# angeris/cfmm-routing-code

Hardware: NVIDIA H100
Metric: pools x dual-evaluations / second (1M constant-product pools, 4096 tokens); time to 1e-6 rel-gap reported beside it (higher is better)
Workload: dtype f64

## Files before the change

### cfmm_routing_code_b200/_lib.py

```python
from __future__ import annotations

import ctypes as C
import os

from . import build as _build

KIND_PRODUCT, KIND_SUM, KIND_GEOMEAN, KIND_BOUNDED = 0, 1, 2, 3

_ERRORS = {
    -1: "CFMM_E_NULL (required pointer is NULL)",
    -2: "CFMM_E_KIND (unknown kind / unsupported arity)",
    -3: "CFMM_E_SIZE (bad size)",
    -4: "CFMM_E_CUDA (CUDA runtime error)",
    -5: "CFMM_E_NODEVICE (no sm_90 device)",
    -6: "CFMM_E_STATE (handle used in the wrong state)",
}


class CfmmError(RuntimeError):
    pass


class Bucket(C.Structure):
    _fields_ = [
        ("kind", C.c_int32), ("arity", C.c_int32), ("n_pools", C.c_int64), ("stride", C.c_int64),
        ("reserves", C.c_void_p), ("tok_idx", C.c_void_p), ("gamma", C.c_void_p),
        ("weights", C.c_void_p), ("logrw", C.c_void_p), ("theta_bar", C.c_void_p),
    ]


class BlockedPairs(C.Structure):
    _fields_ = [
        ("n_pools", C.c_int64), ("n_tiles", C.c_int64), ("pools_per_tile", C.c_int32), ("reserved", C.c_int32),
        ("r0", C.c_void_p), ("r1", C.c_void_p), ("gamma_inv", C.c_void_p), ("lid", C.c_void_p),
        ("pos", C.c_void_p), ("rows", C.c_void_p), ("tok", C.c_void_p), ("desc", C.c_void_p),
    ]


class SolveParams(C.Structure):
    _fields_ = [("tol", C.c_double), ("nu_floor", C.c_double), ("max_iter", C.c_int32), ("cg_max", C.c_int32)]


class SolveResult(C.Structure):
    _fields_ = [("dual_value", C.c_double), ("primal_value", C.c_double), ("gap", C.c_double),
                ("primal_infeas", C.c_double), ("err", C.c_double), ("iters", C.c_int32), ("evals", C.c_int32),
                ("hvps", C.c_int32), ("status", C.c_int32)]


class PeerCtx(C.Structure):
    _fields_ = [("recv_acc_dev", C.c_void_p), ("recv_vec_dev", C.c_void_p), ("rank", C.c_int32), ("world", C.c_int32),
                ("seq_acc", C.c_uint64), ("seq_vec", C.c_uint64)]


class CsrPools(C.Structure):
    _fields_ = [("n_tokens", C.c_int32), ("n_pools", C.c_int64), ("nnz", C.c_int64), ("pool_ptr", C.c_void_p),
                ("tok_idx", C.c_void_p), ("reserves", C.c_void_p), ("weights", C.c_void_p), ("logrw", C.c_void_p),
                ("gamma", C.c_void_p), ("kind", C.c_void_p)]


class Batch(C.Structure):
    _fields_ = [("n_problems", C.c_int32), ("pool_range", C.c_void_p), ("c", C.c_void_p), ("a", C.c_void_p),
                ("flags", C.c_void_p), ("nu", C.c_void_p), ("psi", C.c_void_p), ("stats", C.c_void_p),
                ("delta", C.c_void_p), ("lambda_", C.c_void_p), ("trade_stride", C.c_int64)]


class BatchParams(C.Structure):
    _fields_ = [("tol", C.c_double), ("eps0", C.c_double), ("eps_min", C.c_double), ("eps_shrink", C.c_double),
                ("floor_rel", C.c_double), ("max_outer", C.c_int32), ("max_inner", C.c_int32)]


class EvalOut(C.Structure):
    _fields_ = [("delta", C.c_void_p), ("lambda_", C.c_void_p), ("hcoef", C.c_void_p), ("hmask", C.c_void_p)]


_lib = None


def lib_path() -> str:
    return _build.LIB


def load(build_if_missing: bool = True):
    global _lib
    if _lib is not None:
        return _lib
    path = _build.LIB
    if build_if_missing and _build.needs_build():
        try:
            _build.build_library()
        except Exception as e:
            if not os.path.exists(path):
                raise CfmmError(f"libcfmm_b200.so is missing and could not be built: {e}") from e
    if not os.path.exists(path):
        raise CfmmError("libcfmm_b200.so is missing: run `python -c 'import __graft_entry__ as g; g.build()'`")
    lib = C.CDLL(path)
    vp, i32, i64, dbl = C.c_void_p, C.c_int32, C.c_int64, C.c_double
    lib.cfmm_arb_eval.argtypes = [C.POINTER(Bucket), i32, vp, vp, dbl, vp, vp, C.POINTER(EvalOut), vp]
    lib.cfmm_arb_eval.restype = C.c_int
    for name in ("cfmm_hvp", "cfmm_hess_diag", "cfmm_hess_dense"):
        fn = getattr(lib, name)
        fn.restype = C.c_int
    lib.cfmm_hvp.argtypes = [C.POINTER(Bucket), i32, vp, vp, vp, vp, vp]
    lib.cfmm_hess_diag.argtypes = [C.POINTER(Bucket), i32, vp, vp, vp, vp]
    lib.cfmm_hess_dense.argtypes = [C.POINTER(Bucket), i32, vp, vp, vp, vp]
    lib.cfmm_blocked_layout_info.argtypes = [C.POINTER(i32)] * 4
    lib.cfmm_blocked_layout_info.restype = C.c_int
    lib.cfmm_set_blocked_config.argtypes = [i32]
    lib.cfmm_set_blocked_config.restype = C.c_int
    lib.cfmm_blocked_build_work_bytes.argtypes = [i64]
    lib.cfmm_blocked_build_work_bytes.restype = i64
    lib.cfmm_blocked_build.argtypes = [i64, i32, vp, vp, vp, C.POINTER(BlockedPairs), vp, vp, vp, i64, vp]
    lib.cfmm_blocked_build.restype = C.c_int
    lib.cfmm_blocked_eval.argtypes = [C.POINTER(BlockedPairs), i32, vp, vp, vp, C.POINTER(EvalOut), vp, i64, vp]
    lib.cfmm_blocked_eval.restype = C.c_int
    lib.cfmm_blocked_hvp.argtypes = [C.POINTER(BlockedPairs), i32, vp, vp, vp, vp, vp]
    lib.cfmm_blocked_hvp.restype = C.c_int
    lib.cfmm_blocked_diag.argtypes = [C.POINTER(BlockedPairs), i32, vp, vp, vp]
    lib.cfmm_blocked_diag.restype = C.c_int
    lib.cfmm_blocked_dense.argtypes = [C.POINTER(BlockedPairs), i32, vp, vp, vp]
    lib.cfmm_blocked_dense.restype = C.c_int
    lib.cfmm_blocked_solve_work_bytes.argtypes = [C.POINTER(BlockedPairs), i32]
    lib.cfmm_blocked_solve_work_bytes.restype = i64
    lib.cfmm_blocked_solve.argtypes = [C.POINTER(BlockedPairs), i32, vp, vp, vp, vp, vp, vp, vp,
                                       C.POINTER(SolveParams), C.POINTER(SolveResult), vp]
    lib.cfmm_blocked_solve.restype = C.c_int
    lib.cfmm_blocked_solve_peer.argtypes = [C.POINTER(BlockedPairs), i32, vp, vp, vp, vp, vp, vp, vp,
                                            C.POINTER(SolveParams), C.POINTER(SolveResult), C.POINTER(PeerCtx), vp]
    lib.cfmm_blocked_solve_peer.restype = C.c_int
    lib.cfmm_persist_solve_work_bytes.argtypes = [C.POINTER(BlockedPairs), i32]
    lib.cfmm_persist_solve_work_bytes.restype = i64
    lib.cfmm_persist_solve.argtypes = lib.cfmm_blocked_solve_peer.argtypes
    lib.cfmm_persist_solve.restype = C.c_int
    lib.cfmm_set_persist_cooperative.argtypes = [i32]
    lib.cfmm_set_persist_cooperative.restype = C.c_int
    lib.cfmm_persist_last_profile.argtypes = [vp]
    lib.cfmm_persist_last_profile.restype = C.c_int
    lib.cfmm_batch_solve_work_bytes.argtypes = [C.POINTER(CsrPools), i32, i64]
    lib.cfmm_batch_solve_work_bytes.restype = i64
    lib.cfmm_set_batch_lanes.argtypes = [i32]
    lib.cfmm_set_batch_lanes.restype = C.c_int
    lib.cfmm_batch_solve.argtypes = [C.POINTER(CsrPools), C.POINTER(Batch), C.POINTER(BatchParams), vp, vp]
    lib.cfmm_batch_solve.restype = C.c_int
    lib.cfmm_allreduce_ll.argtypes = [vp, vp, i32, i32, i32, i64, i64, vp, C.c_uint64, vp]
    lib.cfmm_allreduce_ll.restype = C.c_int
    lib.cfmm_sum_update_multipliers.argtypes = [C.POINTER(Bucket), vp, vp, vp, vp]
    lib.cfmm_sum_update_multipliers.restype = C.c_int
    lib.cfmm_zero.argtypes = [vp, i64, vp]
    lib.cfmm_zero.restype = C.c_int
    lib.cfmm_set_scatter_mode.argtypes = [i32]
    lib.cfmm_set_scatter_mode.restype = C.c_int
    lib.cfmm_launch_count.restype = i64
    lib.cfmm_reset_launch_count.restype = None
    lib.cfmm_last_cuda_error.restype = C.c_char_p
    lib.cfmm_version.restype = C.c_char_p
    if os.environ.get("CFMM_BATCH_LANES"):
        lib.cfmm_set_batch_lanes(int(os.environ["CFMM_BATCH_LANES"]))
    if os.environ.get("CFMM_BLOCKED_CFG"):
        for c in os.environ["CFMM_BLOCKED_CFG"].split(","):
            lib.cfmm_set_blocked_config(int(c))
    _lib = lib
    return lib


def check(rc: int, what: str = "cfmm call"):
    if rc != 0:
        extra = ""
        if rc == -4 and _lib is not None:
            extra = ": " + _lib.cfmm_last_cuda_error().decode()
        raise CfmmError(f"{what} failed: {_ERRORS.get(rc, rc)}{extra}")
```

### cfmm_routing_code_b200/csrc/cfmm_blocked.cu

```cuda
#include <math.h>

#include "cfmm_blocked.cuh"

using namespace cfmm;

namespace {

template <int P, int THREADS, int STAGES, int MODE , bool TRADES, bool HESS>
__global__ void __launch_bounds__(THREADS, kCtasPerSm)
k_blocked(const BlockedArgs A) {
    extern __shared__ __align__(128) unsigned char smem_raw[];
    __shared__ uint64_t full[STAGES];
    __shared__ double part[THREADS / 32];
    if (threadIdx.x == 0) {
        for (int s = 0; s < STAGES; ++s) mbar_init(&full[s], 1);
        mbar_fence_init();
    }
    __syncthreads();
    const long long t_beg = (A.n_tiles * (long long)blockIdx.x) / gridDim.x;
    const long long t_end = (A.n_tiles * (long long)(blockIdx.x + 1)) / gridDim.x;
    double acc = 0.0, acc2 = 0.0;
    unsigned phase = 0;
    blocked_pass<P, THREADS, STAGES, MODE, TRADES, HESS, false, true>(A, smem_raw, full, phase, t_beg, t_end, acc, acc2);
    if (MODE == 0) cta_accumulate<THREADS>(acc, part, A.arb);
}

template <int P>
struct __align__(128) TabStage {
    uint32_t rows[BlockedCfg<P>::kRowsMax];
    int32_t tok[BlockedCfg<P>::kTokMax];
    int4 desc;
};

template <int P>
__device__ __forceinline__ void issue_tables(TabStage<P>* st, uint64_t* bar, const BlockedArgs& A, long long tile,
                                             const int4 d) {
    const unsigned rows_b = round16(4u * (unsigned)d.y);
    const unsigned tok_b = round16(4u * (unsigned)d.x);
    mbar_expect_tx(bar, 16u + rows_b + tok_b);
    bulk_g2s(&st->desc, A.desc + tile, 16, bar);
    bulk_g2s(st->rows, A.rows + tile * BlockedCfg<P>::kRowsMax, rows_b, bar);
    bulk_g2s(st->tok, A.tok + tile * BlockedCfg<P>::kTokMax, tok_b, bar);
}

template <int NF>
struct PoolRegs {
    double a[NF];
    uint32_t lid, pos;
};

template <int P, int THREADS, int NF, int NPOOL>
__device__ __forceinline__ void load_pools(PoolRegs<NF> (&r)[NPOOL], const BlockedArgs& A, long long tile, int tid) {
    const long long toff = tile * P;
#pragma unroll
    for (int u = 0; u < NPOOL; ++u) {
        const long long q = toff + tid + u * THREADS;
#pragma unroll
        for (int k = 0; k < NF; ++k) r[u].a[k] = __ldg(A.slab[k] + q);
        r[u].lid = __ldg(A.lid + q);
        r[u].pos = __ldg(A.pos + q);
    }
}

template <int P, int NF>
__device__ __forceinline__ void prefetch_pools_l2(const BlockedArgs& A, long long tile) {
    constexpr int tp = P;
    const long long toff = tile * P;
#pragma unroll
    for (int k = 0; k < NF; ++k) bulk_prefetch_l2(A.slab[k] + toff, tp * 8);
    bulk_prefetch_l2(A.lid + toff, tp * 4);
    bulk_prefetch_l2(A.pos + toff, tp * 4);
}

template <int P, int THREADS, int STAGES, int MODE, bool TRADES, bool HESS>
__global__ void __launch_bounds__(THREADS, kCtasPerSm)
k_blocked_regs(const BlockedArgs A) {
    constexpr int NF = (MODE == 0) ? 3 : 1;
    constexpr int NPOOL = P / THREADS;
    constexpr int NPRE = (P + THREADS - 1) / THREADS;
    using St = TabStage<P>;
    extern __shared__ __align__(128) unsigned char smem_raw[];
    St* stages = reinterpret_cast<St*>(smem_raw);
    double* nul0 = reinterpret_cast<double*>(smem_raw + (size_t)STAGES * sizeof(St));
    double* g0 = nul0 + 2 * P;
    __shared__ uint64_t full[STAGES];
    __shared__ double part[THREADS / 32];
    const int tid = threadIdx.x, lane = tid & 31, warp = tid >> 5;
    const long long t_beg = (A.n_tiles * (long long)blockIdx.x) / gridDim.x;
    const long long t_end = (A.n_tiles * (long long)(blockIdx.x + 1)) / gridDim.x;
    if (tid == 0) {
        for (int s = 0; s < STAGES; ++s) mbar_init(&full[s], 1);
        mbar_fence_init();
    }
    __syncthreads();
    if (tid == 0) {
        for (int s = 0; s < STAGES; ++s) {
            const long long t = t_beg + s;
            if (t < t_end) issue_tables<P>(&stages[s], &full[s], A, t, __ldg(A.desc + t));
        }
        if (t_beg + 1 < t_end) prefetch_pools_l2<P, NF>(A, t_beg + 1);
        if (t_beg + 2 < t_end) prefetch_pools_l2<P, NF>(A, t_beg + 2);
    }
    PoolRegs<NF> cur[NPOOL], nxt[NPOOL];
    if (t_beg < t_end) load_pools<P, THREADS, NF, NPOOL>(cur, A, t_beg, tid);
    asm volatile("griddepcontrol.wait;" ::: "memory");
    asm volatile("griddepcontrol.launch_dependents;" ::: "memory");
    for (int j = blockIdx.x * THREADS + tid; j < A.n_zero; j += gridDim.x * THREADS) A.zero_next[j] = 0.0;
    double acc = 0.0;
    if (t_beg < t_end) {
        mbar_wait(&full[0], 0);
        if (MODE != 2) {
            const int ntok = stages[0].desc.x;
            for (int t = tid; t < ntok; t += THREADS) nul0[t] = __ldg(A.vec + stages[0].tok[t]);
        }
    }
    __syncthreads();
    int stage = 0, pstage = 0, buf = 0;
    unsigned parity = 0;
    for (long long tile = t_beg; tile < t_end; ++tile) {
        St& S = stages[stage];
        const double* nul = nul0 + buf * P;
        double* g = g0 + buf * 2 * P;
        const long long nx = tile + 1;
        int nstage = stage + 1;
        unsigned nparity = parity;
        if (nstage == STAGES) { nstage = 0; nparity ^= 1u; }
        double pre[NPRE];
        int ntok_n = 0;
        if (tid == 0 && tile + 3 < t_end) prefetch_pools_l2<P, NF>(A, tile + 3);
        if (nx < t_end) {
            load_pools<P, THREADS, NF, NPOOL>(nxt, A, nx, tid);
            mbar_wait(&full[nstage], nparity);
            if (MODE != 2) {
                ntok_n = stages[nstage].desc.x;
#pragma unroll
                for (int k = 0; k < NPRE; ++k) {
                    const int t = tid + k * THREADS;
                    pre[k] = (t < ntok_n) ? __ldg(A.vec + stages[nstage].tok[t]) : 0.0;
                }
            }
        }
        {
            double f0[NPOOL], f1[NPOOL];
#pragma unroll
            for (int u = 0; u < NPOOL; ++u) {
                const uint32_t li = cur[u].lid;
                if (MODE == 0) {
                    EvalOp::apply<TRADES, HESS>(A, tile * P + tid + u * THREADS, cur[u].a[0], cur[u].a[NF > 1 ? 1 : 0],
                                                cur[u].a[NF > 2 ? 2 : 0], nul[li & 0xffffu], nul[li >> 16], f0[u], f1[u],
                                                acc);
                } else if (MODE == 1) {
                    f0[u] = cur[u].a[0] * (nul[li & 0xffffu] - nul[li >> 16]);
                    f1[u] = -f0[u];
                } else {
                    f0[u] = cur[u].a[0];
                    f1[u] = f0[u];
                }
            }
#pragma unroll
            for (int u = 0; u < NPOOL; ++u) {
                g[cur[u].pos & 0xffffu] = f0[u];
                g[cur[u].pos >> 16] = f1[u];
            }
        }
        if (MODE != 2 && nx < t_end) {
            double* nn = nul0 + (buf ^ 1) * P;
#pragma unroll
            for (int k = 0; k < NPRE; ++k) {
                const int t = tid + k * THREADS;
                if (t < ntok_n) nn[t] = pre[k];
            }
        }
        __syncthreads();
        if (tid == 0 && tile > t_beg) {
            const long long far = tile - 1 + STAGES;
            if (far < t_end) {
                fence_proxy_async();
                issue_tables<P>(&stages[pstage], &full[pstage], A, far, __ldg(A.desc + far));
            }
        }
        const int nrow = S.desc.y;
        for (int r = tid; r < nrow; r += THREADS) {
            const uint32_t rw = S.rows[r];
            const double* q = g + row_start(rw);
            const int len = row_len(rw);
            double s0 = 0.0, s1 = 0.0;
            int k = 0;
#pragma unroll 1
            for (; k + 4 <= len; k += 4) { s0 += q[k] + q[k + 2]; s1 += q[k + 1] + q[k + 3]; }
            if (k + 2 <= len) { s0 += q[k]; s1 += q[k + 1]; k += 2; }
            if (k < len) s0 += q[k];
            const double s = s0 + s1;
            if (s != 0.0) atomicAdd(A.out + S.tok[row_tok(rw)], s);
        }
#pragma unroll
        for (int u = 0; u < NPOOL; ++u) cur[u] = nxt[u];
        pstage = stage; stage = nstage; parity = nparity; buf ^= 1;
    }
    if (MODE == 0) {
        acc = warp_sum(acc);
        if (lane == 0) part[warp] = acc;
        __syncthreads();
        if (tid < 32) {
            double s = (tid < THREADS / 32) ? part[tid] : 0.0;
            s = warp_sum(s);
            if (tid == 0 && s != 0.0) atomicAdd(A.arb, s);
        }
    }
}

__global__ void __launch_bounds__(256)
k_blocked_dense(long long n_pools, int n, const uint32_t* __restrict__ lid, const int32_t* __restrict__ tok,
                const double* __restrict__ hcoef, double* H) {
    for (long long q = (long long)blockIdx.x * blockDim.x + threadIdx.x; q < n_pools; q += (long long)gridDim.x * blockDim.x) {
        const double h = hcoef[q];
        if (h != 0.0) {
            const long long tile = q / kTileP;
            const uint32_t li = lid[q];
            const long long a = tok[tile * BlockedCfg<kTileP>::kTokMax + (li & 0xffffu)];
            const long long b = tok[tile * BlockedCfg<kTileP>::kTokMax + (li >> 16)];
            atomicAdd(H + a * n + a, h); atomicAdd(H + b * n + b, h);
            atomicAdd(H + a * n + b, -h); atomicAdd(H + b * n + a, -h);
        }
    }
}

int g_pdl = 1;
int g_row_cap = 32;

template <int MODE, bool TRADES, bool HESS>
int launch_tma(const BlockedArgs& A, cudaStream_t st) {
    constexpr int NF = (MODE == 0) ? 3 : 1;
    auto kern = k_blocked<kTileP, kTileT, kTileStages, MODE, TRADES, HESS>;
    const size_t sm = pass_smem_bytes<kTileP, kTileStages>(NF);
    static bool attr = false;
    if (!attr) {
        cudaFuncSetAttribute(kern, cudaFuncAttributeMaxDynamicSharedMemorySize, (int)sm);
        attr = true;
    }
    const long long cap = (long long)kCtasPerSm * num_sms();
    const int grid = (int)(A.n_tiles < cap ? A.n_tiles : cap);
    cudaLaunchConfig_t cfg = {};
    cfg.gridDim = dim3(grid); cfg.blockDim = dim3(kTileT); cfg.dynamicSmemBytes = sm; cfg.stream = st;
    cudaLaunchAttribute at[1];
    at[0].id = cudaLaunchAttributeProgrammaticStreamSerialization;
    at[0].val.programmaticStreamSerializationAllowed = g_pdl;
    cfg.attrs = at; cfg.numAttrs = 1;
    cudaLaunchKernelEx(&cfg, kern, A);
    return check_launch();
}

template <int MODE>
int launch_regs(const BlockedArgs& A, cudaStream_t st) {
    constexpr int P = kTileP, T = kTileT, S = 4;
    auto kern = k_blocked_regs<P, T, S, MODE, false, false>;
    const size_t sm = (size_t)S * sizeof(TabStage<P>) + (size_t)(2 * P + 4 * P) * sizeof(double);
    static bool attr = false;
    if (!attr) {
        cudaFuncSetAttribute(kern, cudaFuncAttributeMaxDynamicSharedMemorySize, (int)sm);
        attr = true;
    }
    const long long cap = (long long)kCtasPerSm * num_sms();
    const int grid = (int)(A.n_tiles < cap ? A.n_tiles : cap);
    cudaLaunchConfig_t cfg = {};
    cfg.gridDim = dim3(grid); cfg.blockDim = dim3(T); cfg.dynamicSmemBytes = sm; cfg.stream = st;
    cudaLaunchAttribute at[1];
    at[0].id = cudaLaunchAttributeProgrammaticStreamSerialization;
    at[0].val.programmaticStreamSerializationAllowed = g_pdl;
    cfg.attrs = at; cfg.numAttrs = 1;
    cudaLaunchKernelEx(&cfg, kern, A);
    return check_launch();
}

}

namespace cfmm {

int fill_blocked_args(const cfmm_blocked_pairs* b, BlockedArgs& A) {
    if (!b) return CFMM_E_NULL;
    if (b->pools_per_tile != kTileP) return CFMM_E_KIND;
    if (b->n_tiles < 0 || b->n_pools < 0 || b->n_pools > b->n_tiles * (int64_t)kTileP) return CFMM_E_SIZE;
    if (b->n_tiles > 0 && (!b->lid || !b->pos || !b->rows || !b->tok || !b->desc)) return CFMM_E_NULL;
    A.n_tiles = b->n_tiles;
    A.M = b->n_tiles * (int64_t)kTileP;
    A.lid = b->lid; A.pos = b->pos; A.rows = b->rows; A.tok = b->tok;
    A.desc = reinterpret_cast<const int4*>(b->desc);
    A.zero_next = nullptr; A.n_zero = 0;
    A.slab[0] = A.slab[1] = A.slab[2] = nullptr;
    A.vec = nullptr; A.vec2 = nullptr; A.beta = 0.0;
    A.out = nullptr; A.arb = nullptr; A.delta = A.lambda = A.hcoef = nullptr;
    return CFMM_OK;
}

}

extern "C" {

int cfmm_blocked_layout_info(int32_t* pools_per_tile, int32_t* rows_stride, int32_t* tok_stride, int32_t* row_cap) {
    if (pools_per_tile) *pools_per_tile = kTileP;
    if (rows_stride) *rows_stride = BlockedCfg<kTileP>::kRowsMax;
    if (tok_stride) *tok_stride = BlockedCfg<kTileP>::kTokMax;
    if (row_cap) *row_cap = g_row_cap;
    return CFMM_OK;
}

int cfmm_set_blocked_config(int32_t cfg) {
    if (cfg >= 300) { const int c = cfg - 300; if (c < 8 || c > 32) return CFMM_E_KIND; g_row_cap = c; return CFMM_OK; }
    if (cfg == 200 || cfg == 201) { g_pdl = cfg - 200; return CFMM_OK; }
    return CFMM_E_KIND;
}

int cfmm_blocked_eval(const cfmm_blocked_pairs* b, int32_t n_tokens, const double* nu, double* psi, double* arb,
                      const cfmm_eval_out* out, double* zero_next, int64_t n_zero, void* stream) {
    BlockedArgs A;
    int rc = fill_blocked_args(b, A);
    if (rc) return rc;
    if (n_tokens <= 0) return CFMM_E_SIZE;
    if (!nu || !psi || !arb) return CFMM_E_NULL;
    if (b->n_tiles == 0) return CFMM_OK;
    if (!b->r0 || !b->r1 || !b->gamma_inv) return CFMM_E_NULL;
    A.slab[0] = b->r0; A.slab[1] = b->r1; A.slab[2] = b->gamma_inv;
    A.vec = nu; A.out = psi; A.arb = arb;
    A.zero_next = zero_next; A.n_zero = zero_next ? (int)n_zero : 0;
    const bool trades = out && out->delta && out->lambda;
    const bool hess = out && out->hcoef;
    if (trades) { A.delta = out->delta; A.lambda = out->lambda; }
    if (hess) A.hcoef = out->hcoef;
    cudaStream_t st = static_cast<cudaStream_t>(stream);
    if (trades && hess) return launch_tma<0, true, true>(A, st);
    if (trades) return launch_tma<0, true, false>(A, st);
    if (hess) return launch_tma<0, false, true>(A, st);
    return launch_tma<0, false, false>(A, st);
}

int cfmm_blocked_hvp(const cfmm_blocked_pairs* b, int32_t n_tokens, const double* hcoef, const double* vt, double* y,
                     double* zero_next, void* stream) {
    BlockedArgs A;
    int rc = fill_blocked_args(b, A);
    if (rc) return rc;
    if (n_tokens <= 0) return CFMM_E_SIZE;
    if (!hcoef || !vt || !y) return CFMM_E_NULL;
    if (b->n_tiles == 0) return CFMM_OK;
    A.slab[0] = hcoef; A.vec = vt; A.out = y;
    A.zero_next = zero_next; A.n_zero = zero_next ? n_tokens : 0;
    return launch_regs<1>(A, static_cast<cudaStream_t>(stream));
}

int cfmm_blocked_dense(const cfmm_blocked_pairs* b, int32_t n_tokens, const double* hcoef, double* H, void* stream) {
    BlockedArgs A;
    int rc = fill_blocked_args(b, A);
    if (rc) return rc;
    if (n_tokens <= 0) return CFMM_E_SIZE;
    if (!hcoef || !H) return CFMM_E_NULL;
    if (b->n_tiles == 0) return CFMM_OK;
    const long long total = b->n_tiles * (long long)kTileP;
    const long long need = (total + 255) / 256, cap = 8LL * num_sms();
    k_blocked_dense<<<(int)(need < cap ? need : cap), 256, 0, static_cast<cudaStream_t>(stream)>>>(total, n_tokens, b->lid, b->tok, hcoef, H);
    return check_launch();
}

int cfmm_blocked_diag(const cfmm_blocked_pairs* b, int32_t n_tokens, const double* hcoef, double* diag, void* stream) {
    BlockedArgs A;
    int rc = fill_blocked_args(b, A);
    if (rc) return rc;
    if (n_tokens <= 0) return CFMM_E_SIZE;
    if (!hcoef || !diag) return CFMM_E_NULL;
    if (b->n_tiles == 0) return CFMM_OK;
    A.slab[0] = hcoef; A.out = diag;
    return launch_regs<2>(A, static_cast<cudaStream_t>(stream));
}

}
```

### cfmm_routing_code_b200/csrc/cfmm_blocked.cuh

```cuda
#pragma once
#include <math.h>

#include "cfmm_dev.cuh"

namespace cfmm {

#ifndef CFMM_TILE_P
#define CFMM_TILE_P 1024
#endif
#ifndef CFMM_CTAS_PER_SM
#define CFMM_CTAS_PER_SM 2
#endif
constexpr int kTileP = CFMM_TILE_P;
constexpr int kTileT = kTileP / 2;
constexpr int kTileStages = 2;
constexpr int kCtasPerSm = CFMM_CTAS_PER_SM;
static_assert(kTileP % 64 == 0 && kTileP <= 1024, "tile size: whole warps of two-pool threads, 10-bit local token ids");

template <int P>
struct BlockedCfg {
    static constexpr int kTokMax = P;
    static constexpr int kRowCapMin = 8;
    static constexpr int kRowsMax = P + 2 * P / kRowCapMin + 8;
};

template <int P, int NF>
struct __align__(128) Stage {
    double a[NF][P];
    uint32_t lid[P];
    uint32_t pos[P];
    uint32_t rows[BlockedCfg<P>::kRowsMax];
    int32_t tok[BlockedCfg<P>::kTokMax];
    int4 desc;
};

struct BlockedArgs {
    long long n_tiles;
    long long M;
    const double* slab[3];
    const uint32_t* lid;
    const uint32_t* pos;
    const uint32_t* rows;
    const int32_t* tok;
    const int4* desc;
    const double* vec;
    const double* vec2;
    double beta;
    double* out;
    double* zero_next;
    int n_zero;
    double* arb;
    double* delta;
    double* lambda;
    double* hcoef;
};

__device__ __forceinline__ unsigned round16(unsigned bytes) { return (bytes + 15u) & ~15u; }

template <int P, int NF>
__device__ __forceinline__ void issue_tile(Stage<P, NF>* st, uint64_t* bar, const BlockedArgs& A, long long tile,
                                           const int4 d) {
    const unsigned rows_b = round16(4u * (unsigned)d.y);
    const unsigned tok_b = round16(4u * (unsigned)d.x);
    const long long off = tile * P;
    mbar_expect_tx(bar, (unsigned)(NF * P * 8 + P * 4 + P * 4 + 16) + rows_b + tok_b);
    bulk_g2s(&st->desc, A.desc + tile, 16, bar);
#pragma unroll
    for (int k = 0; k < NF; ++k) bulk_g2s(st->a[k], A.slab[k] + off, P * 8, bar);
    bulk_g2s(st->lid, A.lid + off, P * 4, bar);
    bulk_g2s(st->pos, A.pos + off, P * 4, bar);
    bulk_g2s(st->rows, A.rows + tile * BlockedCfg<P>::kRowsMax, rows_b, bar);
    bulk_g2s(st->tok, A.tok + tile * BlockedCfg<P>::kTokMax, tok_b, bar);
}

__device__ __forceinline__ double clamp0(double x) {
    const int hi = __double2hiint(x);
    const int m = ~(hi >> 31);
    return __hiloint2double(hi & m, __double2loint(x) & m);
}

struct EvalOp {
    template <bool TRADES, bool HESS>
    __device__ __forceinline__ static void apply(const BlockedArgs& A, long long q, double R0, double R1, double gi,
                                                 double n0, double n1, double& f0, double& f1, double& acc) {
        const double p0 = n0 * R0, p1 = n1 * R1;
        const double w = p0 * p1 * gi;
        const double v = rsqrt(w);
        const double a = p0 * v, b = p1 * v;
        const double ob = 1.0 - b, oa = 1.0 - a;
        const double r0 = fma(-b, gi, 1.0), r1 = fma(-a, gi, 1.0);
        const double x0 = (ob < 0.0) ? ob * gi : clamp0(r0);
        const double x1 = (oa < 0.0) ? oa * gi : clamp0(r1);
        f0 = R0 * x0;
        f1 = R1 * x1;
        acc = fma(n0, f0, fma(n1, f1, acc));
        if (TRADES) {
            A.delta[q] = f0 < 0.0 ? -f0 : 0.0; A.delta[A.M + q] = f1 < 0.0 ? -f1 : 0.0;
            A.lambda[q] = f0 > 0.0 ? f0 : 0.0; A.lambda[A.M + q] = f1 > 0.0 ? f1 : 0.0;
        }
        if (HESS) A.hcoef[q] = (x0 != 0.0 || x1 != 0.0) ? 0.5 * w * v : 0.0;
    }
};

__device__ __forceinline__ int row_start(uint32_t r) { return (int)(r & 0xffffu); }
__device__ __forceinline__ int row_len(uint32_t r) { return (int)((r >> 16) & 0x3fu); }
__device__ __forceinline__ int row_tok(uint32_t r) { return (int)(r >> 22); }

template <bool COHERENT>
__device__ __forceinline__ double load_vec(const double* p) { return COHERENT ? *p : __ldg(p); }
template <int MODE, bool COHERENT>
__device__ __forceinline__ double gather_vec(const BlockedArgs& A, int t) {
    if (MODE == 1 && COHERENT) return fma(A.beta, A.vec[t], A.vec2[t]);
    return load_vec<COHERENT>(A.vec + t);
}

template <int P, int STAGES>
constexpr size_t pass_smem_bytes(int nf) {
    return (size_t)STAGES * (nf == 3 ? sizeof(Stage<P, 3>) : sizeof(Stage<P, 1>)) + (size_t)(3 * P) * sizeof(double);
}

template <int P, int THREADS, int STAGES, int MODE, bool TRADES, bool HESS, bool COHERENT, bool PDL>
__device__ __forceinline__ void blocked_pass(const BlockedArgs& A, unsigned char* smem_raw, uint64_t* full, unsigned& phase,
                                             long long t_beg, long long t_end, double& acc, double& acc2) {
    constexpr int NF = (MODE == 0) ? 3 : 1;
    using St = Stage<P, NF>;
    St* stages = reinterpret_cast<St*>(smem_raw);
    double* nul = reinterpret_cast<double*>(smem_raw + (size_t)STAGES * sizeof(St));
    double* g = nul + P;
    const int tid = threadIdx.x;
    if (tid == 0) {
        for (int s = 0; s < STAGES; ++s) {
            const long long t = t_beg + s;
            if (t < t_end) issue_tile<P, NF>(&stages[s], &full[s], A, t, __ldg(A.desc + t));
        }
    }
    if (PDL) {
        asm volatile("griddepcontrol.wait;" ::: "memory");
        asm volatile("griddepcontrol.launch_dependents;" ::: "memory");
    }
    for (int j = blockIdx.x * THREADS + tid; j < A.n_zero; j += gridDim.x * THREADS) A.zero_next[j] = 0.0;
    int stage = 0;
    constexpr int NPRE = (P + THREADS - 1) / THREADS;
    if (t_beg < t_end) {
        mbar_wait(&full[0], phase & 1u);
        if (MODE != 2) {
            const int ntok = stages[0].desc.x;
            for (int t = tid; t < ntok; t += THREADS) nul[t] = gather_vec<MODE, COHERENT>(A, stages[0].tok[t]);
        }
    }
    __syncthreads();
    for (long long tile = t_beg; tile < t_end; ++tile) {
        St& S = stages[stage];
        phase ^= 1u << stage;
        const int4 d = S.desc;
        const long long far = tile + STAGES;
        int4 dfar = make_int4(0, 0, 0, 0);
        if (tid == 0 && far < t_end) dfar = __ldg(A.desc + far);
        {
            constexpr int NPOOL = P / THREADS;
            double f0[NPOOL], f1[NPOOL];
            uint32_t ps[NPOOL];
#pragma unroll
            for (int u = 0; u < NPOOL; ++u) {
                const int l = tid + u * THREADS;
                const uint32_t li = S.lid[l];
                ps[u] = S.pos[l];
                if (MODE == 0) {
                    EvalOp::apply<TRADES, HESS>(A, tile * P + l, S.a[0][l], S.a[NF > 1 ? 1 : 0][l], S.a[NF > 2 ? 2 : 0][l],
                                                nul[li & 0xffffu], nul[li >> 16], f0[u], f1[u], acc);
                } else if (MODE == 1) {
                    const double pa = nul[li & 0xffffu], pb = nul[li >> 16], h = S.a[0][l];
                    f0[u] = h * (pa - pb);
                    f1[u] = -f0[u];
                    if (COHERENT) {
                        acc = fma(f0[u], pa - pb, acc);
                        acc2 = fma(h, fma(pa, pa, pb * pb), acc2);
                    }
                } else {
                    f0[u] = S.a[0][l];
                    f1[u] = f0[u];
                }
            }
#pragma unroll
            for (int u = 0; u < NPOOL; ++u) {
                g[ps[u] & 0xffffu] = f0[u];
                g[ps[u] >> 16] = f1[u];
            }
        }
        __syncthreads();
        const long long nxt = tile + 1;
        const int nstage = (stage + 1 == STAGES) ? 0 : stage + 1;
        double pre[NPRE];
        int ntok_n = 0;
        if (nxt < t_end) {
            mbar_wait(&full[nstage], (phase >> nstage) & 1u);
            if (MODE != 2) {
                ntok_n = stages[nstage].desc.x;
#pragma unroll
                for (int k = 0; k < NPRE; ++k) {
                    const int t = tid + k * THREADS;
                    pre[k] = (t < ntok_n) ? gather_vec<MODE, COHERENT>(A, stages[nstage].tok[t]) : 0.0;
                }
            }
        }
        for (int r = tid; r < d.y; r += THREADS) {
            const uint32_t rw = S.rows[r];
            const double* q = g + row_start(rw);
            const int len = row_len(rw);
            double s0 = 0.0, s1 = 0.0;
            int k = 0;
#pragma unroll 1
            for (; k + 4 <= len; k += 4) { s0 += q[k] + q[k + 2]; s1 += q[k + 1] + q[k + 3]; }
            if (k + 2 <= len) { s0 += q[k]; s1 += q[k + 1]; k += 2; }
            if (k < len) s0 += q[k];
            const double s = s0 + s1;
            if (s != 0.0) atomicAdd(A.out + S.tok[row_tok(rw)], s);
        }
        if (MODE != 2 && nxt < t_end) {
#pragma unroll
            for (int k = 0; k < NPRE; ++k) {
                const int t = tid + k * THREADS;
                if (t < ntok_n) nul[t] = pre[k];
            }
        }
        __syncthreads();
        if (tid == 0 && far < t_end) {
            fence_proxy_async();
            issue_tile<P, NF>(&S, &full[stage], A, far, dfar);
        }
        stage = nstage;
    }
}

template <int THREADS>
__device__ __forceinline__ void cta_accumulate(double acc, double* part, double* target) {
    const int tid = threadIdx.x;
    acc = warp_sum(acc);
    if ((tid & 31) == 0) part[tid >> 5] = acc;
    __syncthreads();
    if (tid < 32) {
        double s = (tid < THREADS / 32) ? part[tid] : 0.0;
        s = warp_sum(s);
        if (tid == 0 && s != 0.0) atomicAdd(target, s);
    }
}

int fill_blocked_args(const cfmm_blocked_pairs* b, BlockedArgs& A);

}
```

### cfmm_routing_code_b200/csrc/cfmm_layout.cu

```cuda
#include <cub/cub.cuh>

#include "cfmm_blocked.cuh"

using namespace cfmm;

namespace {

constexpr int LT = kTileT;
constexpr int LP = kTileP;
constexpr int LH = 2 * kTileP;
constexpr int LI = 4;
static_assert(LT * LI == LH, "block sort shape");
constexpr int LR = BlockedCfg<kTileP>::kRowsMax;

struct BuildArgs {
    long long m;
    int n_tokens, nb, row_cap, key_bits, tok_bits;
    const int32_t* idx;
    const double* R;
    const double* gamma;
    const uint32_t* order;
    double *r0, *r1, *gi;
    uint32_t *lid, *pos;
    uint32_t* rows;
    int32_t* tok;
    int4* desc;
    int32_t* status;
};

__global__ void __launch_bounds__(256)
k_pool_keys(long long m, int n_tokens, int nb, const int32_t* __restrict__ idx, const double* __restrict__ R,
            const double* __restrict__ gamma, uint32_t* __restrict__ keys, uint32_t* __restrict__ vals, int32_t* status) {
    int bad = 0;
    for (long long i = (long long)blockIdx.x * blockDim.x + threadIdx.x; i < m; i += (long long)gridDim.x * blockDim.x) {
        const int a = idx[2 * i], b = idx[2 * i + 1];
        const double R0 = R[2 * i], R1 = R[2 * i + 1], g = gamma[i];
        const bool ok = a >= 0 && a < n_tokens && b >= 0 && b < n_tokens && a != b && R0 > 0.0 && R1 > 0.0 && isfinite(R0) &&
                        isfinite(R1) && g > 0.0 && g <= 1.0;
        bad |= ok ? 0 : 1;
        const long long ba = ok ? ((long long)a * nb) / n_tokens : 0, bb = ok ? ((long long)b * nb) / n_tokens : 0;
        keys[i] = (uint32_t)((ba * nb + bb) * n_tokens + (ok ? a : 0));
        vals[i] = (uint32_t)i;
    }
    if (__syncthreads_or(bad) && threadIdx.x == 0) atomicAdd(status + 1, 1);
}

using Sort = cub::BlockRadixSort<uint32_t, LT, LI, uint32_t>;
using Scan = cub::BlockScan<int, LT>;

struct TileSmem {
    union { typename Sort::TempStorage sort; typename Scan::TempStorage scan; } tmp;
    uint32_t sk[LH];
    uint32_t sv[LH];
    uint16_t gid[LH];
    int gs[LP + 2];
    int rfirst[LP + 1];
    uint16_t rrank[LR + 8];
    int rstart[LR + 8];
    uint16_t lidh[LP][2], posh[LP][2];
    int ntok, nrow;
};

__global__ void __launch_bounds__(LT)
k_build_tiles(const BuildArgs B) {
    extern __shared__ __align__(16) unsigned char tile_smem_raw[];
    TileSmem& M = *reinterpret_cast<TileSmem*>(tile_smem_raw);
    auto& tmp = M.tmp;
    uint32_t* sk = M.sk; uint32_t* sv = M.sv; uint16_t* gid = M.gid; int* gs = M.gs; int* rfirst = M.rfirst;
    uint32_t* rk = M.sk;
    uint16_t* rrank = M.rrank; int* rstart = M.rstart;
    auto& lidh = M.lidh; auto& posh = M.posh;
    int& s_ntok = M.ntok; int& s_nrow = M.nrow;
    const int tid = threadIdx.x;
    const long long tile = blockIdx.x;
    const long long p0 = tile * LP;
    const int np = (int)(B.m - p0 < LP ? B.m - p0 : LP);
    const int nh = 2 * np;
    uint32_t key[LI], val[LI];
#pragma unroll
    for (int u = 0; u < LI; ++u) {
        const int h = tid * LI + u;
        const int slot = h >= LP ? 1 : 0, l = h - slot * LP;
        if (l < np) {
            const uint32_t pool = B.order[p0 + l];
            key[u] = (uint32_t)B.idx[2 * (long long)pool + slot];
            val[u] = (uint32_t)(slot << 15 | l);
        } else {
            key[u] = 0xffffffffu; val[u] = 0u;
        }
    }
    Sort(tmp.sort).Sort(key, val, 0, 32);
#pragma unroll
    for (int u = 0; u < LI; ++u) { sk[tid * LI + u] = key[u]; sv[tid * LI + u] = val[u]; }
    __syncthreads();
    int head[LI], gpre[LI];
#pragma unroll
    for (int u = 0; u < LI; ++u) {
        const int i = tid * LI + u;
        head[u] = (i < nh && (i == 0 || sk[i] != sk[i - 1])) ? 1 : 0;
    }
    int ntok;
    Scan(tmp.scan).ExclusiveSum(head, gpre, ntok);
    __syncthreads();
    const bool bad = ntok > LP;
#pragma unroll
    for (int u = 0; u < LI; ++u) {
        const int i = tid * LI + u;
        if (i < nh) {
            const int g = gpre[u] + head[u] - 1;
            gid[i] = (uint16_t)g;
            if (head[u] && !bad) { gs[g] = i; B.tok[tile * LP + g] = (int32_t)sk[i]; }
        }
    }
    if (tid == 0) { s_ntok = ntok; if (!bad) gs[ntok] = nh; }
    __syncthreads();
    if (bad) {
        if (tid == 0) { atomicAdd(B.status, 1); B.desc[tile] = make_int4(0, 0, 0, 0); }
        for (int l = tid; l < LP; l += LT) {
            B.r0[p0 + l] = 1.0; B.r1[p0 + l] = 1.0; B.gi[p0 + l] = 1.0; B.lid[p0 + l] = 0u; B.pos[p0 + l] = 0u;
        }
        return;
    }
    const int cap = B.row_cap;
    int nsub[2], rpre[2];
#pragma unroll
    for (int u = 0; u < 2; ++u) {
        const int g = tid * 2 + u;
        nsub[u] = g < ntok ? (gs[g + 1] - gs[g] + cap - 1) / cap : 0;
    }
    int nrow;
    Scan(tmp.scan).ExclusiveSum(nsub, rpre, nrow);
    __syncthreads();
#pragma unroll
    for (int u = 0; u < 2; ++u) {
        const int g = tid * 2 + u;
        if (g < ntok) {
            rfirst[g] = rpre[u];
            const int cnt = gs[g + 1] - gs[g];
            for (int s = 0; s < nsub[u]; ++s) {
                const int len = min(cap, cnt - cap * s);
                rk[rpre[u] + s] = (uint32_t)(63 - len) << 16 | (uint32_t)(rpre[u] + s);
            }
        }
    }
    if (tid == 0) s_nrow = nrow;
    __syncthreads();
    uint32_t rkey[LI], rdum[LI];
#pragma unroll
    for (int u = 0; u < LI; ++u) {
        const int r = tid * LI + u;
        rkey[u] = r < nrow ? rk[r] : 0xffffffffu;
        rdum[u] = 0u;
    }
    __syncthreads();
    Sort(tmp.sort).Sort(rkey, rdum, 0, 22);
    int rlen[LI], spre[LI];
#pragma unroll
    for (int u = 0; u < LI; ++u) {
        const int r = tid * LI + u;
        rlen[u] = r < nrow ? 63 - (int)(rkey[u] >> 16) : 0;
        if (r < nrow) rrank[rkey[u] & 0xffffu] = (uint16_t)r;
    }
    __syncthreads();
    int total;
    Scan(tmp.scan).ExclusiveSum(rlen, spre, total);
#pragma unroll
    for (int u = 0; u < LI; ++u) {
        const int r = tid * LI + u;
        if (r < nrow) { rstart[r] = spre[u]; rk[r] = (uint32_t)rlen[u]; }
    }
    __syncthreads();
    for (int i = tid; i < nh; i += LT) {
        const int g = gid[i], o = i - gs[g];
        const int r = rrank[rfirst[g] + o / cap];
        const int p = rstart[r] + o % cap;
        const uint32_t v = sv[i];
        const int slot = v >> 15, l = v & 0x7fffu;
        lidh[l][slot] = (uint16_t)g;
        posh[l][slot] = (uint16_t)p;
        if (o % cap == 0) B.rows[tile * LR + r] = (uint32_t)rstart[r] | rk[r] << 16 | (uint32_t)g << 22;
    }
    __syncthreads();
    for (int l = tid; l < LP; l += LT) {
        if (l < np) {
            const uint32_t pool = B.order[p0 + l];
            B.lid[p0 + l] = (uint32_t)lidh[l][0] | (uint32_t)lidh[l][1] << 16;
            B.pos[p0 + l] = (uint32_t)posh[l][0] | (uint32_t)posh[l][1] << 16;
            B.r0[p0 + l] = B.R[2 * (long long)pool]; B.r1[p0 + l] = B.R[2 * (long long)pool + 1];
            B.gi[p0 + l] = 1.0 / B.gamma[pool];
        } else {
            const int pl = l - np;
            B.lid[p0 + l] = 0u;
            B.pos[p0 + l] = (uint32_t)(nh + 2 * pl) | (uint32_t)(nh + 2 * pl + 1) << 16;
            B.r0[p0 + l] = 1.0; B.r1[p0 + l] = 1.0; B.gi[p0 + l] = 1.0;
        }
    }
    if (tid == 0) { B.desc[tile] = make_int4(s_ntok, s_nrow, 0, 0); atomicAdd(B.status + 2, s_nrow); }
}

inline size_t align_up(size_t x) { return (x + 255) & ~(size_t)255; }

size_t sort_temp_bytes(long long m) {
    size_t bytes = 0;
    cub::DeviceRadixSort::SortPairs(nullptr, bytes, (const uint32_t*)nullptr, (uint32_t*)nullptr, (const uint32_t*)nullptr,
                                    (uint32_t*)nullptr, (int)m, 0, 32);
    return bytes;
}

}

extern "C" {

int64_t cfmm_blocked_build_work_bytes(int64_t n_pools) {
    if (n_pools <= 0 || n_pools > 0x7fffffffLL) return CFMM_E_SIZE;
    return (int64_t)(4 * align_up(4 * (size_t)n_pools) + align_up(sort_temp_bytes(n_pools)));
}

int cfmm_blocked_build(int64_t n_pools, int32_t n_tokens, const int32_t* idx, const double* reserves, const double* gamma,
                       const cfmm_blocked_pairs* out, uint32_t* order, int32_t* status, void* work, int64_t work_bytes,
                       void* stream) {
    if (!idx || !reserves || !gamma || !out || !order || !status || !work) return CFMM_E_NULL;
    if (n_pools <= 0 || n_pools > 0x7fffffffLL || n_tokens <= 0) return CFMM_E_SIZE;
    if (work_bytes < cfmm_blocked_build_work_bytes(n_pools)) return CFMM_E_SIZE;
    const long long T = (n_pools + LP - 1) / LP;
    if (out->pools_per_tile != LP || out->n_tiles != T || out->n_pools != n_pools) return CFMM_E_SIZE;
    if (!out->r0 || !out->r1 || !out->gamma_inv || !out->lid || !out->pos || !out->rows || !out->tok || !out->desc) return CFMM_E_NULL;
    int row_cap = 32;
    cfmm_blocked_layout_info(nullptr, nullptr, nullptr, &row_cap);
    long long nb = (long long)llround(sqrt((double)n_pools / LP));
    if (nb < 1) nb = 1;
    if ((double)nb * nb * n_tokens >= 4294967296.0) return CFMM_E_SIZE;
    int key_bits = 1;
    while (key_bits < 32 && (1ull << key_bits) < (unsigned long long)(nb * nb) * (unsigned long long)n_tokens) ++key_bits;
    cudaStream_t st = static_cast<cudaStream_t>(stream);
    unsigned char* w = static_cast<unsigned char*>(work);
    auto take = [&](size_t bytes) { unsigned char* p = w; w += align_up(bytes); return p; };
    uint32_t* keys = reinterpret_cast<uint32_t*>(take(4 * (size_t)n_pools));
    uint32_t* vals = reinterpret_cast<uint32_t*>(take(4 * (size_t)n_pools));
    uint32_t* keys2 = reinterpret_cast<uint32_t*>(take(4 * (size_t)n_pools));
    take(4 * (size_t)n_pools);
    size_t temp_bytes = sort_temp_bytes(n_pools);
    void* temp = take(temp_bytes);
    cudaMemsetAsync(status, 0, 16, st);
    const int grid = (int)((n_pools + 255) / 256 < 4LL * num_sms() ? (n_pools + 255) / 256 : 4LL * num_sms());
    k_pool_keys<<<grid, 256, 0, st>>>(n_pools, n_tokens, (int)nb, idx, reserves, gamma, keys, vals, status);
    int rc = check_launch();
    if (rc) return rc;
    if (cub::DeviceRadixSort::SortPairs(temp, temp_bytes, keys, keys2, vals, order, (int)n_pools, 0, key_bits, st) != cudaSuccess) {
        g_last_err = cudaGetLastError();
        return CFMM_E_CUDA;
    }
    BuildArgs B;
    B.m = n_pools; B.n_tokens = n_tokens; B.nb = (int)nb; B.row_cap = row_cap; B.key_bits = key_bits; B.tok_bits = 32;
    B.idx = idx; B.R = reserves; B.gamma = gamma; B.order = order;
    B.r0 = const_cast<double*>(out->r0); B.r1 = const_cast<double*>(out->r1); B.gi = const_cast<double*>(out->gamma_inv);
    B.lid = const_cast<uint32_t*>(out->lid); B.pos = const_cast<uint32_t*>(out->pos);
    B.rows = const_cast<uint32_t*>(out->rows); B.tok = const_cast<int32_t*>(out->tok);
    B.desc = reinterpret_cast<int4*>(const_cast<int32_t*>(out->desc));
    B.status = status;
    static bool attr = false;
    if (!attr) {
        cudaFuncSetAttribute(k_build_tiles, cudaFuncAttributeMaxDynamicSharedMemorySize, (int)sizeof(TileSmem));
        attr = true;
    }
    k_build_tiles<<<(int)T, LT, sizeof(TileSmem), st>>>(B);
    return check_launch();
}

}
```

### cfmm_routing_code_b200/pools.py

```python
from __future__ import annotations

import ctypes as C
import dataclasses
from typing import Dict, List, Optional, Sequence

import numpy as np
import torch

from . import _lib

KIND_GEOMEAN_HOST = 0
KIND_SUM_HOST = 1
KIND_BOUNDED_HOST = 3


@dataclasses.dataclass
class HostPools:
    n_tokens: int
    pool_ptr: np.ndarray
    tok_idx: np.ndarray
    reserves: np.ndarray
    weights: np.ndarray
    gamma: np.ndarray
    kind: np.ndarray

    @property
    def m(self) -> int:
        return int(len(self.gamma))

    @staticmethod
    def from_lists(n_tokens, local_indices, reserves, fees, kinds, weights=None) -> "HostPools":
        m = len(local_indices)
        if not (len(reserves) == len(fees) == len(kinds) == m):
            raise ValueError("local_indices, reserves, fees, kinds must have one entry per pool")
        ptr = [0]; idx: List[int] = []; res: List[float] = []; wts: List[float] = []; kd: List[int] = []
        for i, l in enumerate(local_indices):
            k = len(l)
            if len(reserves[i]) != k:
                raise ValueError(f"pool {i}: {len(reserves[i])} reserves for {k} tokens")
            if len(set(int(t) for t in l)) != k:
                raise ValueError(f"pool {i}: repeated token in local_indices")
            ptr.append(ptr[-1] + k)
            idx += [int(t) for t in l]
            res += [float(x) for x in reserves[i]]
            if kinds[i] == "sum":
                if k != 2:
                    raise ValueError("constant-sum pools must have 2 tokens (as arbitrage.py:11)")
                kd.append(KIND_SUM_HOST); wts += [0.0] * k
            elif kinds[i] == "bounded_product":
                o = None if (weights is None or weights[i] is None) else np.asarray(weights[i], float)
                if k != 2 or o is None or len(o) != 2 or np.any(o < 0) or not np.all(np.isfinite(o)):
                    raise ValueError(f"pool {i}: bounded_product needs 2 tokens and 2 non-negative offsets in weights[i]")
                kd.append(KIND_BOUNDED_HOST); wts += list(o)
            elif kinds[i] in ("geomean", "product"):
                w = np.ones(k) if (weights is None or weights[i] is None) else np.asarray(weights[i], float)
                if len(w) != k or np.any(w <= 0):
                    raise ValueError(f"pool {i}: bad weights")
                kd.append(KIND_GEOMEAN_HOST); wts += list(w / w.sum())
            else:
                raise ValueError(f"pool {i}: unknown kind {kinds[i]!r}")
        return HostPools(int(n_tokens), np.asarray(ptr, np.int64), np.asarray(idx, np.int32),
                         np.asarray(res, np.float64), np.asarray(wts, np.float64),
                         np.asarray(fees, np.float64), np.asarray(kd, np.uint8))

    @staticmethod
    def from_pairs(n_tokens, idx, reserves, gamma) -> "HostPools":
        m = len(gamma)
        hp = HostPools(int(n_tokens), np.arange(0, 2 * m + 1, 2, dtype=np.int64),
                       np.ascontiguousarray(idx, np.int32).reshape(-1),
                       np.ascontiguousarray(reserves, np.float64).reshape(-1),
                       np.full(2 * m, 0.5), np.ascontiguousarray(gamma, np.float64), np.zeros(m, np.uint8))
        hp._uniform_product = True
        return hp

    def pin_memory(self) -> "HostPools":
        keep = []
        for name in ("tok_idx", "reserves", "weights", "gamma", "kind", "pool_ptr"):
            t = torch.from_numpy(np.ascontiguousarray(getattr(self, name))).pin_memory()
            keep.append(t)
            setattr(self, name, t.numpy())
        self._pinned = keep
        return self

    def validate(self):
        slot_kind = np.repeat(np.asarray(self.kind), np.diff(self.pool_ptr)) if np.any(self.kind == KIND_BOUNDED_HOST) else None
        virt = self.reserves if slot_kind is None else self.reserves + np.where(slot_kind == KIND_BOUNDED_HOST, self.weights, 0.0)
        lo_ok = np.all(self.reserves > 0) if slot_kind is None else np.all(self.reserves >= 0) and np.all(virt > 0)
        if not lo_ok or not np.all(np.isfinite(self.reserves)):
            raise ValueError("reserves must be positive and finite (bounded_product: >= 0 with positive virtual reserves)")
        if np.any(self.gamma <= 0) or np.any(self.gamma > 1):
            raise ValueError("fees (gamma) must lie in (0, 1]")
        if self.tok_idx.min(initial=0) < 0 or self.tok_idx.max(initial=0) >= self.n_tokens:
            raise ValueError("token index out of range")


class BucketSpec:

    def __init__(self, hp: HostPools, kind: int, arity: int, sel: Optional[np.ndarray], lo: int = 0,
                 hi: Optional[int] = None):
        self.hp, self.kind, self.arity, self._sel = hp, kind, arity, sel
        self.lo, self.hi = int(lo), int(hp.m if hi is None else hi)
        self._contiguous = sel is None
        self.m = (self.hi - self.lo) if sel is None else int(len(sel))
        self._off = None

    @property
    def identity(self) -> bool:
        return self._contiguous

    @property
    def sel(self) -> np.ndarray:
        if self._sel is None:
            self._sel = np.arange(self.lo, self.hi, dtype=np.int64)
        return self._sel

    @property
    def off(self) -> np.ndarray:
        if self._off is None:
            self._off = self.hp.pool_ptr[self.sel][None, :] + np.arange(self.arity)[:, None]
        return self._off

    def subset(self, local_idx: np.ndarray) -> "BucketSpec":
        return BucketSpec(self.hp, self.kind, self.arity, self.sel[local_idx])


def split_buckets(hp: HostPools, rank: int = 0, world: int = 1) -> List["BucketSpec"]:
    m = hp.m
    if m == 0:
        return []
    if getattr(hp, "_uniform_product", False):
        lo, hi = (m * rank) // world, (m * (rank + 1)) // world
        return [BucketSpec(hp, _lib.KIND_PRODUCT, 2, None, lo, hi)]
    uniform_pairs = int(hp.pool_ptr[-1]) == 2 * m and (hp.pool_ptr[1] - hp.pool_ptr[0]) == 2 and \
        bool(np.all(np.diff(hp.pool_ptr[::max(1, m // 64)]) == 2 * max(1, m // 64))) and \
        bool(np.array_equal(hp.pool_ptr[:3], np.arange(0, 2 * min(m, 2) + 1, 2)[:3]))
    if uniform_pairs:
        uniform_pairs = bool(np.all(np.diff(hp.pool_ptr) == 2))
    if uniform_pairs and not hp.kind.any() and bool(np.all(hp.weights == 0.5)):
        lo, hi = (m * rank) // world, (m * (rank + 1)) // world
        return [BucketSpec(hp, _lib.KIND_PRODUCT, 2, None, lo, hi)]
    ar = np.diff(hp.pool_ptr)
    first = hp.pool_ptr[:-1]
    is_cp = (hp.kind == KIND_GEOMEAN_HOST) & (ar == 2)
    is_cp &= (hp.weights[first] == 0.5) & (hp.weights[np.minimum(first + 1, len(hp.weights) - 1)] == 0.5)
    keys = []
    if is_cp.any():
        keys.append((_lib.KIND_PRODUCT, 2, np.nonzero(is_cp)[0]))
    cs = hp.kind == KIND_SUM_HOST
    if cs.any():
        if np.any(ar[cs] != 2):
            raise ValueError("constant-sum pools must have 2 tokens")
        keys.append((_lib.KIND_SUM, 2, np.nonzero(cs)[0]))
    bp = hp.kind == KIND_BOUNDED_HOST
    if bp.any():
        if np.any(ar[bp] != 2):
            raise ValueError("bounded_product pools must have 2 tokens")
        keys.append((_lib.KIND_BOUNDED, 2, np.nonzero(bp)[0]))
    gm = (hp.kind == KIND_GEOMEAN_HOST) & ~is_cp
    for k in np.unique(ar[gm]).tolist():
        if k < 2 or k > 32:
            raise ValueError(f"weighted pools support 2..32 tokens, got {k}")
        keys.append((_lib.KIND_GEOMEAN, int(k), np.nonzero(gm & (ar == k))[0]))
    out = []
    for kind, k, sel in keys:
        if world > 1:
            lo = (len(sel) * rank) // world
            hi = (len(sel) * (rank + 1)) // world
            sel = sel[lo:hi]
        out.append(BucketSpec(hp, kind, k, sel))
    return out


TILE = 1024


def _padded(arr2d: np.ndarray, stride: int, fill) -> np.ndarray:
    k, m = arr2d.shape
    out = np.full((k, stride), fill, dtype=arr2d.dtype)
    out[:, :m] = arr2d
    return out


class DeviceBucket:
    def __init__(self, hp: HostPools, spec, device):
        self.kind = spec.kind; self.arity = spec.arity
        self.spec = spec
        self.m = spec.m
        self.stride = max(TILE, -(-self.m // TILE) * TILE)
        f64 = dict(dtype=torch.float64, device=device)
        self.weights = self.logrw = self.theta_bar = None
        if spec.identity and self.arity == 2 and int(hp.pool_ptr[-1]) == 2 * hp.m:
            m, lo, hi = self.m, spec.lo, spec.hi
            self.reserves = torch.ones((2, self.stride), **f64)
            self.reserves[:, :m] = torch.from_numpy(hp.reserves[2 * lo:2 * hi]).to(device).view(m, 2).t()
            self.tok_idx = torch.zeros((2, self.stride), dtype=torch.int32, device=device)
            self.tok_idx[:, :m] = torch.from_numpy(hp.tok_idx[2 * lo:2 * hi]).to(device).view(m, 2).t()
            self.gamma = torch.ones(self.stride, **f64)
            self.gamma[:m] = torch.from_numpy(hp.gamma[lo:hi]).to(device)
            R = W = None
        else:
            R = hp.reserves[spec.off]
            self.reserves = torch.as_tensor(_padded(R, self.stride, 1.0), **f64)
            self.tok_idx = torch.as_tensor(_padded(hp.tok_idx[spec.off].astype(np.int32), self.stride, 0),
                                           dtype=torch.int32, device=device)
            self.gamma = torch.as_tensor(_padded(hp.gamma[spec.sel][None, :], self.stride, 1.0)[0], **f64)
        if self.kind == _lib.KIND_GEOMEAN:
            W = hp.weights[spec.off]
            self.weights = torch.as_tensor(_padded(W, self.stride, 1.0), **f64)
            self.logrw = torch.as_tensor(_padded(np.log(R / W), self.stride, 0.0), **f64)
        if self.kind == _lib.KIND_BOUNDED:
            self.weights = torch.as_tensor(_padded(hp.weights[spec.off], self.stride, 1.0), **f64)
        if self.kind == _lib.KIND_SUM:
            self.theta_bar = torch.zeros((2, self.stride), **f64)
        self.delta = self.lam = self.hcoef = self.hmask = None
        self._device = device
        self.c_bucket = _lib.Bucket(
            self.kind, self.arity, self.m, self.stride, self.reserves.data_ptr(), self.tok_idx.data_ptr(),
            self.gamma.data_ptr(),
            self.weights.data_ptr() if self.weights is not None else None,
            self.logrw.data_ptr() if self.logrw is not None else None,
            self.theta_bar.data_ptr() if self.theta_bar is not None else None)

    @property
    def sel(self) -> np.ndarray:
        return self.spec.sel

    @property
    def off(self) -> np.ndarray:
        return self.spec.off

    def bytes_resident(self) -> int:
        n = 0
        for t in (self.reserves, self.tok_idx, self.gamma, self.weights, self.logrw, self.theta_bar):
            if t is not None:
                n += t.numel() * t.element_size()
        return n

    def out_struct(self, trades: bool, hess: bool):
        f64 = dict(dtype=torch.float64, device=self._device)
        if trades and self.delta is None:
            self.delta = torch.zeros((self.arity, self.stride), **f64)
            self.lam = torch.zeros((self.arity, self.stride), **f64)
        if hess and self.hcoef is None:
            self.hcoef = torch.zeros(self.stride, **f64)
            self.hmask = torch.zeros(self.stride, dtype=torch.int32, device=self._device)
        return _lib.EvalOut(self.delta.data_ptr() if trades else None, self.lam.data_ptr() if trades else None,
                            self.hcoef.data_ptr() if hess else None, self.hmask.data_ptr() if hess else None)


def blocked_layout_info(lib):
    v = [C.c_int32() for _ in range(4)]
    _lib.check(lib.cfmm_blocked_layout_info(*[C.byref(x) for x in v]), "cfmm_blocked_layout_info")
    return tuple(int(x.value) for x in v)


def build_blocked_pairs(idx: torch.Tensor, n_tokens: int, P: int, rows_stride: int, tok_stride: int, row_cap: int):
    dev = idx.device
    m = idx.shape[1]
    i64 = dict(dtype=torch.int64, device=dev)
    nb = max(1, int(round((m / P) ** 0.5)))
    a, b = idx[0], idx[1]
    key = ((a * nb // n_tokens) * nb + (b * nb // n_tokens)) * n_tokens + a
    order = torch.argsort(key, stable=True)
    residual = []
    for _pass in range(4):
        mm = order.numel()
        if mm == 0:
            break
        pos = torch.arange(mm, **i64)
        ntiles = -(-mm // P)
        tile = pos // P
        he_tok = torch.cat([a[order], b[order]])
        he_tile = torch.cat([tile, tile])
        ck, perm = torch.sort(he_tile * n_tokens + he_tok, stable=True)
        uniq, inv, counts = torch.unique_consecutive(ck, return_inverse=True, return_counts=True)
        u_tile = uniq // n_tokens
        ntok = torch.bincount(u_tile, minlength=ntiles)
        bad = ntok > tok_stride
        if not bool(bad.any()):
            break
        if _pass == 3:
            residual.append(order); order = order[:0]; mm = 0
            break
        keep = ~bad[tile]
        residual.append(order[~keep])
        order = order[keep]
    residual = torch.cat(residual) if residual else order[:0]
    if order.numel() == 0:
        return order, residual, None
    U = uniq.numel()
    tok_off = torch.cumsum(ntok, 0) - ntok
    ltok_u = torch.arange(U, **i64) - tok_off[u_tile]
    he_ltok = torch.empty(2 * mm, **i64)
    he_ltok[perm] = ltok_u[inv]
    M = ntiles * P
    lid = torch.zeros(M, dtype=torch.int32, device=dev)
    lid[:mm] = (he_ltok[:mm] | (he_ltok[mm:] << 16)).to(torch.int32)
    tok = torch.zeros((ntiles, tok_stride), dtype=torch.int32, device=dev)
    tok[u_tile, ltok_u] = (uniq - u_tile * n_tokens).to(torch.int32)
    nsub = (counts + row_cap - 1) // row_cap
    n_rows = int(nsub.sum())
    first_row_u = torch.cumsum(nsub, 0) - nsub
    row_u = torch.repeat_interleave(torch.arange(U, **i64), nsub)
    sub = torch.arange(n_rows, **i64) - first_row_u[row_u]
    g_start = torch.cumsum(counts, 0) - counts
    row_tile0 = u_tile[row_u]
    row_len0 = torch.clamp(counts[row_u] - row_cap * sub, max=row_cap)
    srt = torch.argsort(row_tile0 * 64 + (63 - row_len0), stable=True)
    rank = torch.empty_like(srt); rank[srt] = torch.arange(n_rows, **i64)
    row_tile, row_len, row_ltok = row_tile0[srt], row_len0[srt], ltok_u[row_u][srt]
    nrow = torch.bincount(row_tile, minlength=ntiles)
    row_first = torch.cumsum(nrow, 0) - nrow
    r_local = torch.arange(n_rows, **i64) - row_first[row_tile]
    if int(nrow.max()) > rows_stride:
        raise _lib.CfmmError("blocked layout: row table overflow (library/builder mismatch)")
    cs = torch.cumsum(row_len, 0) - row_len
    row_start = cs - cs[row_first][row_tile]
    he_o = torch.arange(2 * mm, **i64) - g_start[inv]
    he_row = rank[first_row_u[inv] + he_o // row_cap]
    he_pos = torch.empty(2 * mm, **i64)
    he_pos[perm] = row_start[he_row] + he_o % row_cap
    pos = torch.zeros(M, dtype=torch.int32, device=dev)
    pad_base = 2 * (mm - (ntiles - 1) * P)
    if M > mm:
        padl = torch.arange(M - mm, **i64)
        pos[mm:] = ((pad_base + 2 * padl) | ((pad_base + 2 * padl + 1) << 16)).to(torch.int32)
    pos[:mm] = (he_pos[:mm] | (he_pos[mm:] << 16)).to(torch.int32)
    rows = torch.zeros((ntiles, rows_stride), dtype=torch.int32, device=dev)
    word = row_start | (row_len << 16) | (row_ltok << 22)
    rows[row_tile, r_local] = torch.where(word >= 2 ** 31, word - 2 ** 32, word).to(torch.int32)
    desc = torch.stack([ntok, nrow, torch.zeros_like(ntok), torch.zeros_like(ntok)], 1).to(torch.int32).contiguous()
    tables = dict(n_tiles=ntiles, M=M, lid=lid, tok=tok, pos=pos, rows=rows, desc=desc,
                  rows_per_pool=n_rows / mm, tok_per_tile=float(ntok.double().mean()))
    return order, residual, tables


class BlockedBucket:
    kind = _lib.KIND_PRODUCT
    arity = 2
    blocked = True

    def __init__(self, hp: HostPools, spec, device, lib):
        self.spec = spec
        P, rows_stride, tok_stride, row_cap = blocked_layout_info(lib)
        f64 = dict(dtype=torch.float64, device=device)
        self.theta_bar = None
        self.delta = self.lam = self.hcoef = self.hmask = None
        self._device = device
        self._sel = self._off = None
        if spec.identity and int(hp.pool_ptr[-1]) == 2 * hp.m and self._build_native(hp, spec, device, lib, P, rows_stride, tok_stride):
            return
        if spec.identity:
            lo, hi = spec.lo, spec.hi
            R = torch.from_numpy(hp.reserves[2 * lo:2 * hi]).to(device, non_blocking=True).view(-1, 2)
            idx = torch.from_numpy(hp.tok_idx[2 * lo:2 * hi]).to(device, non_blocking=True).view(-1, 2).to(torch.int64)
            gam = torch.from_numpy(hp.gamma[lo:hi]).to(device, non_blocking=True)
            if getattr(hp, "_validate_on_device", False):
                chk = torch.stack([R.min(), gam.min(), 1.0 - gam.max(), idx.min().double(),
                                   float(hp.n_tokens - 1) - idx.max().double(),
                                   torch.isfinite(R).all().double() - 0.5]).cpu()
                if bool((chk[:2] <= 0).any()) or bool((chk[2:] < 0).any()):
                    raise ValueError("invalid pool data (reserves > 0, fees in (0, 1], token ids in range, finite)")
        else:
            R = torch.as_tensor(np.ascontiguousarray(hp.reserves[spec.off].T), **f64)
            idx = torch.as_tensor(np.ascontiguousarray(hp.tok_idx[spec.off].T).astype(np.int64), device=device)
            gam = torch.as_tensor(np.ascontiguousarray(hp.gamma[spec.sel]), **f64)
        order, residual, t = build_blocked_pairs(idx.t(), hp.n_tokens, P, rows_stride, tok_stride, row_cap)
        self.order = order
        self.residual = residual.cpu().numpy() if residual.numel() else np.zeros(0, np.int64)
        self.m = int(order.numel())
        if self.m == 0:
            self.tables = None
            return
        self.tables = t
        self.stride = t["M"]

        def slab(vals, fill):
            out = torch.full((t["M"],), fill, **f64)
            out[:self.m] = vals
            return out
        self.r0 = slab(R[order, 0], 1.0)
        self.r1 = slab(R[order, 1], 1.0)
        self.gamma_inv = slab(1.0 / gam[order], 1.0)
        self.c_blocked = _lib.BlockedPairs(self.m, t["n_tiles"], P, 0, self.r0.data_ptr(), self.r1.data_ptr(),
                                           self.gamma_inv.data_ptr(), t["lid"].data_ptr(), t["pos"].data_ptr(),
                                           t["rows"].data_ptr(), t["tok"].data_ptr(), t["desc"].data_ptr())

    def _build_native(self, hp, spec, device, lib, P, rows_stride, tok_stride) -> bool:
        lo, hi = spec.lo, spec.hi
        m = hi - lo
        if m <= 0:
            return False
        nb = max(1, int(round((m / P) ** 0.5)))
        if nb * nb * hp.n_tokens >= 2 ** 32 or m >= 2 ** 31:
            return False
        T = -(-m // P)
        M = T * P
        f64 = dict(dtype=torch.float64, device=device)
        i32 = dict(dtype=torch.int32, device=device)
        idx = torch.from_numpy(np.ascontiguousarray(hp.tok_idx[2 * lo:2 * hi], np.int32)).to(device, non_blocking=True)
        R = torch.from_numpy(hp.reserves[2 * lo:2 * hi]).to(device, non_blocking=True)
        gam = torch.from_numpy(hp.gamma[lo:hi]).to(device, non_blocking=True)
        slabs = torch.empty((3, M), **f64)
        words = torch.empty((2, M), **i32)
        rows = torch.empty((T, rows_stride), **i32)
        tok = torch.empty((T, tok_stride), **i32)
        desc = torch.empty((T, 4), **i32)
        order = torch.empty(m, **i32)
        status = torch.empty(4, **i32)
        nbytes = int(lib.cfmm_blocked_build_work_bytes(m))
        if nbytes <= 0:
            return False
        work = torch.empty(nbytes, dtype=torch.uint8, device=device)
        cb = _lib.BlockedPairs(m, T, P, 0, slabs[0].data_ptr(), slabs[1].data_ptr(), slabs[2].data_ptr(), words[0].data_ptr(),
                               words[1].data_ptr(), rows.data_ptr(), tok.data_ptr(), desc.data_ptr())
        st = C.c_void_p(torch.cuda.current_stream(device).cuda_stream)
        rc = lib.cfmm_blocked_build(m, hp.n_tokens, idx.data_ptr(), R.data_ptr(), gam.data_ptr(), C.byref(cb), order.data_ptr(),
                                    status.data_ptr(), work.data_ptr(), nbytes, st)
        if rc == -3:
            return False
        _lib.check(rc, "cfmm_blocked_build")
        st_h = status.cpu()
        if int(st_h[1]) != 0:
            raise ValueError("invalid pool data (reserves > 0 and finite, fees in (0, 1], two distinct token ids in range)")
        if int(st_h[0]) != 0:
            return False
        self.order = order
        self.residual = np.zeros(0, np.int64)
        self.m = m
        self.stride = M
        self.r0, self.r1, self.gamma_inv = slabs[0], slabs[1], slabs[2]
        self._keep = (idx, R, gam, work)
        self.tables = dict(n_tiles=T, M=M, lid=words[0], pos=words[1], rows=rows, tok=tok, desc=desc,
                           rows_per_pool=int(st_h[2]) / m, tok_per_tile=None)
        self.c_blocked = cb
        return True

    @property
    def sel(self) -> np.ndarray:
        if self._sel is None:
            self._sel = self.spec.sel[self.order.cpu().numpy().astype(np.int64)]
        return self._sel

    @property
    def off(self) -> np.ndarray:
        if self._off is None:
            self._off = self.spec.hp.pool_ptr[self.sel][None, :] + np.arange(2)[:, None]
        return self._off

    def bytes_resident(self) -> int:
        if self.tables is None:
            return 0
        ts = [self.r0, self.r1, self.gamma_inv] + [self.tables[k] for k in ("lid", "tok", "pos", "rows", "desc")]
        return sum(x.numel() * x.element_size() for x in ts)

    def out_struct(self, trades: bool, hess: bool):
        f64 = dict(dtype=torch.float64, device=self._device)
        if trades and self.delta is None:
            self.delta = torch.zeros((2, self.stride), **f64)
            self.lam = torch.zeros((2, self.stride), **f64)
        if hess and self.hcoef is None:
            self.hcoef = torch.zeros(self.stride, **f64)
        return _lib.EvalOut(self.delta.data_ptr() if trades else None, self.lam.data_ptr() if trades else None,
                            self.hcoef.data_ptr() if hess else None, None)


class PeerContext:

    def __init__(self, n_tokens: int, device, group):
        import torch.distributed as dist
        import torch.distributed._symmetric_memory as symm
        n = int(n_tokens)
        if n + 1 > 64 * 256:
            raise _lib.CfmmError("peer all-reduce supports n_tokens < 16384; use NCCL (Comm) beyond that")
        f64 = dict(dtype=torch.float64, device=device)
        self.group = group
        self.rank, self.world = dist.get_rank(group), dist.get_world_size(group)
        self.n_tokens = n
        w = self.world
        self.sym_acc = symm.empty((3 * w * (n + 1) * 2,), **f64); self.sym_acc.zero_()
        self.sym_y = symm.empty((3 * w * (n + 2) * 2,), **f64); self.sym_y.zero_()
        self.hdl_acc = symm.rendezvous(self.sym_acc, group)
        self.hdl_y = symm.rendezvous(self.sym_y, group)
        self.red_acc = torch.zeros(n + 1, **f64)
        self.red_y = torch.zeros(n, **f64)
        self.seq = [0, 0]
        torch.cuda.synchronize(device)
        dist.barrier(group)

    def next_seq(self, chan: int) -> int:
        self.seq[chan] += 1
        return self.seq[chan]

    def c_struct(self):
        return _lib.PeerCtx(int(self.hdl_acc.buffer_ptrs_dev), int(self.hdl_y.buffer_ptrs_dev), self.rank, self.world,
                            self.seq[0], self.seq[1])

    def absorb(self, c):
        self.seq = [int(c.seq_acc), int(c.seq_vec)]


_PEER_CONTEXTS: Dict[tuple, "PeerContext"] = {}


def peer_context(n_tokens: int, device, group=None) -> "PeerContext":
    import torch.distributed as dist
    group = group or dist.group.WORLD
    key = (int(n_tokens), id(group), str(torch.device(device)))
    if key not in _PEER_CONTEXTS:
        _PEER_CONTEXTS[key] = PeerContext(n_tokens, torch.device(device), group)
    return _PEER_CONTEXTS[key]


class PoolStore:

    def __init__(self, hp: HostPools, device="cuda", rank: int = 0, world: int = 1, validate: bool = True,
                 layout: str = "blocked"):
        if layout not in ("blocked", "plain"):
            raise ValueError("layout must be 'blocked' or 'plain'")
        if validate:
            if getattr(hp, "_uniform_product", False) and layout == "blocked":
                hp._validate_on_device = True
            else:
                hp.validate()
        self.lib = _lib.load()
        self.device = torch.device(device)
        if self.device.type != "cuda":
            raise _lib.CfmmError("PoolStore needs a CUDA device: there is no CPU path in this package")
        if not torch.cuda.is_available():
            raise _lib.CfmmError("no CUDA device visible: the routing kernels have no CPU fallback")
        self.n_tokens = int(hp.n_tokens)
        self.m_total = hp.m
        self.pool_ptr = hp.pool_ptr
        self._tok_idx_host = hp.tok_idx
        self.rank, self.world = rank, world
        self.buckets = []
        for s in split_buckets(hp, rank, world):
            if s.kind == _lib.KIND_PRODUCT and layout == "blocked" and s.m > 0:
                bb = BlockedBucket(hp, s, self.device, self.lib)
                if bb.m > 0:
                    self.buckets.append(bb)
                if len(bb.residual):
                    self.buckets.append(DeviceBucket(hp, s.subset(bb.residual), self.device))
            else:
                self.buckets.append(DeviceBucket(hp, s, self.device))
        self.buckets.sort(key=lambda b: 0 if getattr(b, "blocked", False) else 1)
        self._blocked_first = bool(self.buckets) and getattr(self.buckets[0], "blocked", False)
        assert sum(1 for b in self.buckets if getattr(b, "blocked", False)) <= 1
        self.m_local = sum(b.m for b in self.buckets)
        self.has_sum = bool(np.any(hp.kind == KIND_SUM_HOST))
        self.has_geomean = any(b.kind == _lib.KIND_GEOMEAN for b in self.buckets)
        f64 = dict(dtype=torch.float64, device=self.device)
        self._acc2 = torch.zeros((2, self.n_tokens + 1), **f64)
        self._y2 = torch.zeros((2, self.n_tokens), **f64)
        self._acc_i = 0
        self._y_i = 0
        self._move = torch.zeros(1, **f64)
        self.evals = 0
        self.hvps = 0

    def enable_peer_allreduce(self, group=None):
        self._peer = peer_context(self.n_tokens, self.device, group)
        self.reduces_internally = True

    def _peer_reduce(self, chan, local, n, st):
        p = self._peer
        seq = p.next_seq(chan)
        hdl, out = (p.hdl_acc, p.red_acc) if chan == 0 else (p.hdl_y, p.red_y)
        _lib.check(self.lib.cfmm_allreduce_ll(local.data_ptr(), int(hdl.buffer_ptrs_dev), p.rank, p.world, n,
                                              (seq % 3) * p.world * n, n, out.data_ptr(), seq, st), "cfmm_allreduce_ll")
        return out

    def _stream(self):
        return C.c_void_p(torch.cuda.current_stream(self.device).cuda_stream)

    def bytes_resident(self) -> int:
        return sum(b.bytes_resident() for b in self.buckets)

    def algorithmic_bytes_per_eval(self) -> int:
        n = 0
        for b in self.buckets:
            n += b.m * (28 * b.arity + 12 if b.kind == _lib.KIND_GEOMEAN else 48 if b.kind == _lib.KIND_BOUNDED else 32)
        return n + 16 * self.n_tokens + 8

    def evaluate(self, nu: torch.Tensor, eps: float = 0.0, trades: bool = False, hess: bool = False, reduce: bool = True):
        st = self._stream()
        acc = self._acc2[self._acc_i]
        nxt = self._acc2[self._acc_i ^ 1]
        self._acc_i ^= 1
        if not self._blocked_first:
            _lib.check(self.lib.cfmm_zero(acc.data_ptr(), acc.numel() * 8, st), "cfmm_zero")
        lognu = torch.log(nu) if self.has_geomean else None
        for b in self.buckets:
            out = b.out_struct(trades, hess) if (trades or hess) else None
            if getattr(b, "blocked", False):
                rc = self.lib.cfmm_blocked_eval(C.byref(b.c_blocked), self.n_tokens, nu.data_ptr(), acc.data_ptr(),
                                                acc.data_ptr() + 8 * self.n_tokens,
                                                C.byref(out) if out is not None else None,
                                                nxt.data_ptr(), nxt.numel(), st)
                _lib.check(rc, "cfmm_blocked_eval")
                continue
            rc = self.lib.cfmm_arb_eval(C.byref(b.c_bucket), self.n_tokens, nu.data_ptr(),
                                        lognu.data_ptr() if lognu is not None else None, float(eps),
                                        acc.data_ptr(), acc.data_ptr() + 8 * self.n_tokens,
                                        C.byref(out) if out is not None else None, st)
            _lib.check(rc, "cfmm_arb_eval")
        self.evals += 1
        if reduce and getattr(self, "reduces_internally", False):
            return self._peer_reduce(0, acc, self.n_tokens + 1, st)
        return acc

    def hvp(self, vt: torch.Tensor) -> torch.Tensor:
        st = self._stream()
        y = self._y2[self._y_i]
        ynxt = self._y2[self._y_i ^ 1]
        self._y_i ^= 1
        if not self._blocked_first:
            _lib.check(self.lib.cfmm_zero(y.data_ptr(), y.numel() * 8, st), "cfmm_zero")
        for b in self.buckets:
            if getattr(b, "blocked", False):
                _lib.check(self.lib.cfmm_blocked_hvp(C.byref(b.c_blocked), self.n_tokens, b.hcoef.data_ptr(),
                                                     vt.data_ptr(), y.data_ptr(), ynxt.data_ptr(), st),
                           "cfmm_blocked_hvp")
                continue
            rc = self.lib.cfmm_hvp(C.byref(b.c_bucket), self.n_tokens, b.hcoef.data_ptr(),
                                   b.hmask.data_ptr(), vt.data_ptr(), y.data_ptr(), st)
            _lib.check(rc, "cfmm_hvp")
        self.hvps += 1
        if getattr(self, "reduces_internally", False):
            return self._peer_reduce(1, y, self.n_tokens, st)
        return y

    def hess_diag(self) -> torch.Tensor:
        st = self._stream()
        d = torch.zeros(self.n_tokens, dtype=torch.float64, device=self.device)
        for b in self.buckets:
            if getattr(b, "blocked", False):
                _lib.check(self.lib.cfmm_blocked_diag(C.byref(b.c_blocked), self.n_tokens, b.hcoef.data_ptr(),
                                                      d.data_ptr(), st), "cfmm_blocked_diag")
                continue
            _lib.check(self.lib.cfmm_hess_diag(C.byref(b.c_bucket), self.n_tokens, b.hcoef.data_ptr(),
                                               b.hmask.data_ptr(), d.data_ptr(), st), "cfmm_hess_diag")
        if getattr(self, "reduces_internally", False):
            return self._peer_reduce(1, d, self.n_tokens, st).clone()
        return d

    def hess_dense(self) -> torch.Tensor:
        st = self._stream()
        H = torch.zeros((self.n_tokens, self.n_tokens), dtype=torch.float64, device=self.device)
        for b in self.buckets:
            if getattr(b, "blocked", False):
                _lib.check(self.lib.cfmm_blocked_dense(C.byref(b.c_blocked), self.n_tokens, b.hcoef.data_ptr(), H.data_ptr(), st),
                           "cfmm_blocked_dense")
                continue
            _lib.check(self.lib.cfmm_hess_dense(C.byref(b.c_bucket), self.n_tokens, b.hcoef.data_ptr(),
                                                b.hmask.data_ptr(), H.data_ptr(), st), "cfmm_hess_dense")
        return H

    def update_multipliers(self) -> torch.Tensor:
        st = self._stream()
        self._move.zero_()
        for b in self.buckets:
            if b.kind == _lib.KIND_SUM:
                _lib.check(self.lib.cfmm_sum_update_multipliers(C.byref(b.c_bucket), b.lam.data_ptr(),
                                                                b.theta_bar.data_ptr(), self._move.data_ptr(), st),
                           "cfmm_sum_update_multipliers")
        return self._move

    def reset_multipliers(self):
        for b in self.buckets:
            if b.theta_bar is not None:
                b.theta_bar.zero_()

    def gather_trades(self):
        nnz = int(self.pool_ptr[-1])
        delta = np.zeros(nnz); lam = np.zeros(nnz)
        for b in self.buckets:
            if b.m == 0:
                continue
            delta[b.off.ravel()] = b.delta[:, :b.m].cpu().numpy().ravel()
            lam[b.off.ravel()] = b.lam[:, :b.m].cpu().numpy().ravel()
        return delta, lam
```

### include/cfmm_b200.h

```cpp
#ifndef CFMM_B200_H
#define CFMM_B200_H

#include <stdint.h>

#ifdef __cplusplus
extern "C" {
#endif

enum {
    CFMM_KIND_PRODUCT = 0,
    CFMM_KIND_SUM = 1,
    CFMM_KIND_GEOMEAN = 2,
    CFMM_KIND_BOUNDED_PRODUCT = 3
};

enum {
    CFMM_OK = 0,
    CFMM_E_NULL = -1,
    CFMM_E_KIND = -2,
    CFMM_E_SIZE = -3,
    CFMM_E_CUDA = -4,
    CFMM_E_NODEVICE = -5,
    CFMM_E_STATE = -6
};

typedef struct cfmm_bucket {
    int32_t kind;
    int32_t arity;
    int64_t n_pools;
    int64_t stride;
    const double* reserves;
    const int32_t* tok_idx;
    const double* gamma;
    const double* weights;
    const double* logrw;
    const double* theta_bar;
} cfmm_bucket;

typedef struct cfmm_eval_out {
    double* delta;
    double* lambda;
    double* hcoef;
    uint32_t* hmask;
} cfmm_eval_out;

int cfmm_arb_eval(const cfmm_bucket* bucket, int32_t n_tokens, const double* nu, const double* log_nu,
                  double eps, double* psi, double* arb, const cfmm_eval_out* out, void* stream);

int cfmm_hvp(const cfmm_bucket* bucket, int32_t n_tokens, const double* hcoef, const uint32_t* hmask,
             const double* vt, double* y, void* stream);

int cfmm_hess_diag(const cfmm_bucket* bucket, int32_t n_tokens, const double* hcoef, const uint32_t* hmask,
                   double* diag, void* stream);

int cfmm_hess_dense(const cfmm_bucket* bucket, int32_t n_tokens, const double* hcoef, const uint32_t* hmask,
                    double* H, void* stream);

typedef struct cfmm_blocked_pairs {
    int64_t n_pools;
    int64_t n_tiles;
    int32_t pools_per_tile;
    int32_t reserved;
    const double* r0;
    const double* r1;
    const double* gamma_inv;
    const uint32_t* lid;
    const uint32_t* pos;
    const uint32_t* rows;
    const int32_t* tok;
    const int32_t* desc;
} cfmm_blocked_pairs;

int cfmm_blocked_layout_info(int32_t* pools_per_tile, int32_t* rows_stride, int32_t* tok_stride, int32_t* row_cap);
int cfmm_set_blocked_config(int32_t cfg);

int64_t cfmm_blocked_build_work_bytes(int64_t n_pools);
int cfmm_blocked_build(int64_t n_pools, int32_t n_tokens, const int32_t* idx, const double* reserves, const double* gamma,
                       const cfmm_blocked_pairs* out, uint32_t* order, int32_t* status, void* work, int64_t work_bytes,
                       void* stream);

int cfmm_blocked_eval(const cfmm_blocked_pairs* b, int32_t n_tokens, const double* nu, double* psi, double* arb,
                      const cfmm_eval_out* out, double* zero_next, int64_t n_zero, void* stream);
int cfmm_blocked_hvp(const cfmm_blocked_pairs* b, int32_t n_tokens, const double* hcoef, const double* vt, double* y,
                     double* zero_next, void* stream);
int cfmm_blocked_diag(const cfmm_blocked_pairs* b, int32_t n_tokens, const double* hcoef, double* diag, void* stream);
int cfmm_blocked_dense(const cfmm_blocked_pairs* b, int32_t n_tokens, const double* hcoef, double* H, void* stream);

typedef struct cfmm_solve_params {
    double tol;
    double nu_floor;
    int32_t max_iter;
    int32_t cg_max;
} cfmm_solve_params;

typedef struct cfmm_solve_result {
    double dual_value, primal_value, gap, primal_infeas, err;
    int32_t iters, evals, hvps, status;
} cfmm_solve_result;

int64_t cfmm_blocked_solve_work_bytes(const cfmm_blocked_pairs* b, int32_t n_tokens);
int cfmm_blocked_solve(const cfmm_blocked_pairs* b, int32_t n_tokens, const double* c, const double* a,
                       const uint8_t* eq, const uint8_t* pinned, double* nu, double* psi_out, void* work,
                       const cfmm_solve_params* prm, cfmm_solve_result* res, void* stream);

typedef struct cfmm_peer_ctx {
    const void* recv_acc_dev;
    const void* recv_vec_dev;
    int32_t rank, world;
    uint64_t seq_acc, seq_vec;
} cfmm_peer_ctx;

int cfmm_blocked_solve_peer(const cfmm_blocked_pairs* b, int32_t n_tokens, const double* c, const double* a,
                            const uint8_t* eq, const uint8_t* pinned, double* nu, double* psi_out, void* work,
                            const cfmm_solve_params* prm, cfmm_solve_result* res, cfmm_peer_ctx* peer, void* stream);

int64_t cfmm_persist_solve_work_bytes(const cfmm_blocked_pairs* b, int32_t n_tokens);
int cfmm_set_persist_cooperative(int32_t on);
int cfmm_persist_last_profile(int64_t* out8);
int cfmm_persist_solve(const cfmm_blocked_pairs* b, int32_t n_tokens, const double* c, const double* a,
                       const uint8_t* eq, const uint8_t* pinned, double* nu, double* psi_out, void* work,
                       const cfmm_solve_params* prm, cfmm_solve_result* res, cfmm_peer_ctx* peer, void* stream);

typedef struct cfmm_csr_pools {
    int32_t n_tokens;
    int64_t n_pools, nnz;
    const int64_t* pool_ptr;
    const int32_t* tok_idx;
    const double* reserves;
    const double* weights;
    const double* logrw;
    const double* gamma;
    const uint8_t* kind;
} cfmm_csr_pools;

typedef struct cfmm_batch {
    int32_t n_problems;
    const int64_t* pool_range;
    const double* c;
    const double* a;
    const uint8_t* flags;
    double* nu;
    double* psi;
    double* stats;
    double* delta;
    double* lambda;
    int64_t trade_stride;
} cfmm_batch;

typedef struct cfmm_batch_params {
    double tol;
    double eps0, eps_min, eps_shrink;
    double floor_rel;
    int32_t max_outer, max_inner;
} cfmm_batch_params;

int64_t cfmm_batch_solve_work_bytes(const cfmm_csr_pools* pools, int32_t n_problems, int64_t nnz_max);
int cfmm_set_batch_lanes(int32_t lanes);
int cfmm_batch_solve(const cfmm_csr_pools* pools, const cfmm_batch* batch, const cfmm_batch_params* prm, void* work,
                     void* stream);

int cfmm_allreduce_ll(const double* local, const void* peer_recv_dev, int32_t rank, int32_t world, int32_t n,
                      int64_t slot_off_cells, int64_t src_stride_cells, double* out, uint64_t seq, void* stream);

int cfmm_sum_update_multipliers(const cfmm_bucket* bucket, const double* lambda, double* theta_bar_out,
                                double* move, void* stream);

int cfmm_zero(void* ptr, int64_t bytes, void* stream);

int cfmm_set_scatter_mode(int32_t mode);

int64_t cfmm_launch_count(void);
void cfmm_reset_launch_count(void);
const char* cfmm_last_cuda_error(void);
const char* cfmm_version(void);

#ifdef __cplusplus
}
#endif
#endif
```

Measured before the change: 55.75 billion.

## Pack pool local-token ids and scatter position into one 32-bit word

Replaces the two per-pool uint32 arrays (lid, pos) with a single packed word holding two 10-bit local token ids and a 10-bit position for the second half-edge. The first half-edge is now written at a fixed slot (its pool index), so only the second needs a position. The tile builder is reworked on device and in torch to produce this layout. Per-pool index traffic and shared-memory stage size shrink by 4 bytes per pool, which matters in a bandwidth-bound f64 kernel. In exchange, tiles are capped at 1024 pools and the ABI struct changes.

```diff
diff --git a/cfmm_routing_code_b200/_lib.py b/cfmm_routing_code_b200/_lib.py
--- a/cfmm_routing_code_b200/_lib.py
+++ b/cfmm_routing_code_b200/_lib.py
@@ -32,8 +32,8 @@
 class BlockedPairs(C.Structure):
     _fields_ = [
         ("n_pools", C.c_int64), ("n_tiles", C.c_int64), ("pools_per_tile", C.c_int32), ("reserved", C.c_int32),
-        ("r0", C.c_void_p), ("r1", C.c_void_p), ("gamma_inv", C.c_void_p), ("lid", C.c_void_p),
-        ("pos", C.c_void_p), ("rows", C.c_void_p), ("tok", C.c_void_p), ("desc", C.c_void_p),
+        ("r0", C.c_void_p), ("r1", C.c_void_p), ("gamma_inv", C.c_void_p), ("pw", C.c_void_p),
+        ("reserved_ptr", C.c_void_p), ("rows", C.c_void_p), ("tok", C.c_void_p), ("desc", C.c_void_p),
     ]
 
 
diff --git a/cfmm_routing_code_b200/csrc/cfmm_blocked.cu b/cfmm_routing_code_b200/csrc/cfmm_blocked.cu
--- a/cfmm_routing_code_b200/csrc/cfmm_blocked.cu
+++ b/cfmm_routing_code_b200/csrc/cfmm_blocked.cu
@@ -46,7 +46,7 @@
 template <int NF>
 struct PoolRegs {
     double a[NF];
-    uint32_t lid, pos;
+    uint32_t pw;
 };
 
 template <int P, int THREADS, int NF, int NPOOL>
@@ -57,8 +57,7 @@
         const long long q = toff + tid + u * THREADS;
 #pragma unroll
         for (int k = 0; k < NF; ++k) r[u].a[k] = __ldg(A.slab[k] + q);
-        r[u].lid = __ldg(A.lid + q);
-        r[u].pos = __ldg(A.pos + q);
+        r[u].pw = __ldg(A.pw + q);
     }
 }
 
@@ -68,8 +67,7 @@
     const long long toff = tile * P;
 #pragma unroll
     for (int k = 0; k < NF; ++k) bulk_prefetch_l2(A.slab[k] + toff, tp * 8);
-    bulk_prefetch_l2(A.lid + toff, tp * 4);
-    bulk_prefetch_l2(A.pos + toff, tp * 4);
+    bulk_prefetch_l2(A.pw + toff, tp * 4);
 }
 
 template <int P, int THREADS, int STAGES, int MODE, bool TRADES, bool HESS>
@@ -144,13 +142,13 @@
             double f0[NPOOL], f1[NPOOL];
 #pragma unroll
             for (int u = 0; u < NPOOL; ++u) {
-                const uint32_t li = cur[u].lid;
+                const uint32_t w = cur[u].pw;
                 if (MODE == 0) {
                     EvalOp::apply<TRADES, HESS>(A, tile * P + tid + u * THREADS, cur[u].a[0], cur[u].a[NF > 1 ? 1 : 0],
-                                                cur[u].a[NF > 2 ? 2 : 0], nul[li & 0xffffu], nul[li >> 16], f0[u], f1[u],
+                                                cur[u].a[NF > 2 ? 2 : 0], nul[pw_lid0(w)], nul[pw_lid1(w)], f0[u], f1[u],
                                                 acc);
                 } else if (MODE == 1) {
-                    f0[u] = cur[u].a[0] * (nul[li & 0xffffu] - nul[li >> 16]);
+                    f0[u] = cur[u].a[0] * (nul[pw_lid0(w)] - nul[pw_lid1(w)]);
                     f1[u] = -f0[u];
                 } else {
                     f0[u] = cur[u].a[0];
@@ -159,8 +157,8 @@
             }
 #pragma unroll
             for (int u = 0; u < NPOOL; ++u) {
-                g[cur[u].pos & 0xffffu] = f0[u];
-                g[cur[u].pos >> 16] = f1[u];
+                g[tid + u * THREADS] = f0[u];
+                g[P + pw_pos1(cur[u].pw)] = f1[u];
             }
         }
         if (MODE != 2 && nx < t_end) {
@@ -210,15 +208,15 @@
 }
 
 __global__ void __launch_bounds__(256)
-k_blocked_dense(long long n_pools, int n, const uint32_t* __restrict__ lid, const int32_t* __restrict__ tok,
+k_blocked_dense(long long n_pools, int n, const uint32_t* __restrict__ pw, const int32_t* __restrict__ tok,
                 const double* __restrict__ hcoef, double* H) {
     for (long long q = (long long)blockIdx.x * blockDim.x + threadIdx.x; q < n_pools; q += (long long)gridDim.x * blockDim.x) {
         const double h = hcoef[q];
         if (h != 0.0) {
             const long long tile = q / kTileP;
-            const uint32_t li = lid[q];
-            const long long a = tok[tile * BlockedCfg<kTileP>::kTokMax + (li & 0xffffu)];
-            const long long b = tok[tile * BlockedCfg<kTileP>::kTokMax + (li >> 16)];
+            const uint32_t w = pw[q];
+            const long long a = tok[tile * BlockedCfg<kTileP>::kTokMax + pw_lid0(w)];
+            const long long b = tok[tile * BlockedCfg<kTileP>::kTokMax + pw_lid1(w)];
             atomicAdd(H + a * n + a, h); atomicAdd(H + b * n + b, h);
             atomicAdd(H + a * n + b, -h); atomicAdd(H + b * n + a, -h);
         }
@@ -280,10 +278,11 @@
     if (!b) return CFMM_E_NULL;
     if (b->pools_per_tile != kTileP) return CFMM_E_KIND;
     if (b->n_tiles < 0 || b->n_pools < 0 || b->n_pools > b->n_tiles * (int64_t)kTileP) return CFMM_E_SIZE;
-    if (b->n_tiles > 0 && (!b->lid || !b->pos || !b->rows || !b->tok || !b->desc)) return CFMM_E_NULL;
+    if (b->reserved_ptr) return CFMM_E_KIND;
+    if (b->n_tiles > 0 && (!b->pw || !b->rows || !b->tok || !b->desc)) return CFMM_E_NULL;
     A.n_tiles = b->n_tiles;
     A.M = b->n_tiles * (int64_t)kTileP;
-    A.lid = b->lid; A.pos = b->pos; A.rows = b->rows; A.tok = b->tok;
+    A.pw = b->pw; A.rows = b->rows; A.tok = b->tok;
     A.desc = reinterpret_cast<const int4*>(b->desc);
     A.zero_next = nullptr; A.n_zero = 0;
     A.slab[0] = A.slab[1] = A.slab[2] = nullptr;
@@ -355,7 +354,7 @@
     if (b->n_tiles == 0) return CFMM_OK;
     const long long total = b->n_tiles * (long long)kTileP;
     const long long need = (total + 255) / 256, cap = 8LL * num_sms();
-    k_blocked_dense<<<(int)(need < cap ? need : cap), 256, 0, static_cast<cudaStream_t>(stream)>>>(total, n_tokens, b->lid, b->tok, hcoef, H);
+    k_blocked_dense<<<(int)(need < cap ? need : cap), 256, 0, static_cast<cudaStream_t>(stream)>>>(total, n_tokens, b->pw, b->tok, hcoef, H);
     return check_launch();
 }
 
diff --git a/cfmm_routing_code_b200/csrc/cfmm_blocked.cuh b/cfmm_routing_code_b200/csrc/cfmm_blocked.cuh
--- a/cfmm_routing_code_b200/csrc/cfmm_blocked.cuh
+++ b/cfmm_routing_code_b200/csrc/cfmm_blocked.cuh
@@ -15,7 +15,11 @@
 constexpr int kTileT = kTileP / 2;
 constexpr int kTileStages = 2;
 constexpr int kCtasPerSm = CFMM_CTAS_PER_SM;
-static_assert(kTileP % 64 == 0 && kTileP <= 1024, "tile size: whole warps of two-pool threads, 10-bit local token ids");
+static_assert(kTileP % 64 == 0 && kTileP <= 1024, "tile size: whole warps of two-pool threads, 10-bit fields of the pool word");
+
+__device__ __forceinline__ int pw_lid0(uint32_t w) { return (int)(w & 0x3ffu); }
+__device__ __forceinline__ int pw_lid1(uint32_t w) { return (int)((w >> 10) & 0x3ffu); }
+__device__ __forceinline__ int pw_pos1(uint32_t w) { return (int)(w >> 20); }
 
 template <int P>
 struct BlockedCfg {
@@ -27,8 +31,7 @@
 template <int P, int NF>
 struct __align__(128) Stage {
     double a[NF][P];
-    uint32_t lid[P];
-    uint32_t pos[P];
+    uint32_t pw[P];
     uint32_t rows[BlockedCfg<P>::kRowsMax];
     int32_t tok[BlockedCfg<P>::kTokMax];
     int4 desc;
@@ -38,8 +41,7 @@
     long long n_tiles;
     long long M;
     const double* slab[3];
-    const uint32_t* lid;
-    const uint32_t* pos;
+    const uint32_t* pw;
     const uint32_t* rows;
     const int32_t* tok;
     const int4* desc;
@@ -63,12 +65,11 @@
     const unsigned rows_b = round16(4u * (unsigned)d.y);
     const unsigned tok_b = round16(4u * (unsigned)d.x);
     const long long off = tile * P;
-    mbar_expect_tx(bar, (unsigned)(NF * P * 8 + P * 4 + P * 4 + 16) + rows_b + tok_b);
+    mbar_expect_tx(bar, (unsigned)(NF * P * 8 + P * 4 + 16) + rows_b + tok_b);
     bulk_g2s(&st->desc, A.desc + tile, 16, bar);
 #pragma unroll
     for (int k = 0; k < NF; ++k) bulk_g2s(st->a[k], A.slab[k] + off, P * 8, bar);
-    bulk_g2s(st->lid, A.lid + off, P * 4, bar);
-    bulk_g2s(st->pos, A.pos + off, P * 4, bar);
+    bulk_g2s(st->pw, A.pw + off, P * 4, bar);
     bulk_g2s(st->rows, A.rows + tile * BlockedCfg<P>::kRowsMax, rows_b, bar);
     bulk_g2s(st->tok, A.tok + tile * BlockedCfg<P>::kTokMax, tok_b, bar);
 }
@@ -159,17 +160,17 @@
         {
             constexpr int NPOOL = P / THREADS;
             double f0[NPOOL], f1[NPOOL];
-            uint32_t ps[NPOOL];
+            uint32_t ws[NPOOL];
 #pragma unroll
             for (int u = 0; u < NPOOL; ++u) {
                 const int l = tid + u * THREADS;
-                const uint32_t li = S.lid[l];
-                ps[u] = S.pos[l];
+                const uint32_t w = S.pw[l];
+                ws[u] = w;
                 if (MODE == 0) {
                     EvalOp::apply<TRADES, HESS>(A, tile * P + l, S.a[0][l], S.a[NF > 1 ? 1 : 0][l], S.a[NF > 2 ? 2 : 0][l],
-                                                nul[li & 0xffffu], nul[li >> 16], f0[u], f1[u], acc);
+                                                nul[pw_lid0(w)], nul[pw_lid1(w)], f0[u], f1[u], acc);
                 } else if (MODE == 1) {
-                    const double pa = nul[li & 0xffffu], pb = nul[li >> 16], h = S.a[0][l];
+                    const double pa = nul[pw_lid0(w)], pb = nul[pw_lid1(w)], h = S.a[0][l];
                     f0[u] = h * (pa - pb);
                     f1[u] = -f0[u];
                     if (COHERENT) {
@@ -183,8 +184,8 @@
             }
 #pragma unroll
             for (int u = 0; u < NPOOL; ++u) {
-                g[ps[u] & 0xffffu] = f0[u];
-                g[ps[u] >> 16] = f1[u];
+                g[tid + u * THREADS] = f0[u];
+                g[P + pw_pos1(ws[u])] = f1[u];
             }
         }
         __syncthreads();
diff --git a/cfmm_routing_code_b200/csrc/cfmm_layout.cu b/cfmm_routing_code_b200/csrc/cfmm_layout.cu
--- a/cfmm_routing_code_b200/csrc/cfmm_layout.cu
+++ b/cfmm_routing_code_b200/csrc/cfmm_layout.cu
@@ -21,11 +21,15 @@
     const double* gamma;
     const uint32_t* order;
     double *r0, *r1, *gi;
-    uint32_t *lid, *pos;
+    uint32_t* pw;
     uint32_t* rows;
     int32_t* tok;
     int4* desc;
     int32_t* status;
+};
+
+struct MaxOp {
+    __device__ __forceinline__ int operator()(int a, int b) const { return a > b ? a : b; }
 };
 
 __global__ void __launch_bounds__(256)
@@ -53,29 +57,34 @@
     uint32_t sk[LH];
     uint32_t sv[LH];
     uint16_t gid[LH];
-    int gs[LP + 2];
-    int rfirst[LP + 1];
-    uint16_t rrank[LR + 8];
-    int rstart[LR + 8];
-    uint16_t lidh[LP][2], posh[LP][2];
-    int ntok, nrow;
+    uint16_t ftok[LH];
+    uint16_t rlen[LH];
+    uint16_t lidh[LP][2], p1h[LP];
+    int ntok;
 };
+
+__device__ void inert_tile(const BuildArgs& B, long long tile) {
+    const long long p0 = tile * LP;
+    if (threadIdx.x == 0) { atomicAdd(B.status, 1); B.desc[tile] = make_int4(0, 0, 0, 0); }
+    for (int l = threadIdx.x; l < LP; l += LT) {
+        B.r0[p0 + l] = 1.0; B.r1[p0 + l] = 1.0; B.gi[p0 + l] = 1.0; B.pw[p0 + l] = 0u;
+    }
+}
 
 __global__ void __launch_bounds__(LT)
 k_build_tiles(const BuildArgs B) {
     extern __shared__ __align__(16) unsigned char tile_smem_raw[];
     TileSmem& M = *reinterpret_cast<TileSmem*>(tile_smem_raw);
     auto& tmp = M.tmp;
-    uint32_t* sk = M.sk; uint32_t* sv = M.sv; uint16_t* gid = M.gid; int* gs = M.gs; int* rfirst = M.rfirst;
-    uint32_t* rk = M.sk;
-    uint16_t* rrank = M.rrank; int* rstart = M.rstart;
-    auto& lidh = M.lidh; auto& posh = M.posh;
-    int& s_ntok = M.ntok; int& s_nrow = M.nrow;
+    uint32_t* sk = M.sk; uint32_t* sv = M.sv; uint16_t* gid = M.gid; uint16_t* ftok = M.ftok; uint16_t* rlen = M.rlen;
+    auto& lidh = M.lidh; uint16_t* p1h = M.p1h;
+    int& s_ntok = M.ntok;
     const int tid = threadIdx.x;
     const long long tile = blockIdx.x;
     const long long p0 = tile * LP;
     const int np = (int)(B.m - p0 < LP ? B.m - p0 : LP);
     const int nh = 2 * np;
+    auto real = [&](int c) { return (c < LP ? c : c - LP) < np; };
     uint32_t key[LI], val[LI];
 #pragma unroll
     for (int u = 0; u < LI; ++u) {
@@ -102,100 +111,84 @@
     int ntok;
     Scan(tmp.scan).ExclusiveSum(head, gpre, ntok);
     __syncthreads();
-    const bool bad = ntok > LP;
+    if (ntok > LP) { inert_tile(B, tile); return; }
 #pragma unroll
     for (int u = 0; u < LI; ++u) {
         const int i = tid * LI + u;
         if (i < nh) {
             const int g = gpre[u] + head[u] - 1;
             gid[i] = (uint16_t)g;
-            if (head[u] && !bad) { gs[g] = i; B.tok[tile * LP + g] = (int32_t)sk[i]; }
-        }
-    }
-    if (tid == 0) { s_ntok = ntok; if (!bad) gs[ntok] = nh; }
-    __syncthreads();
-    if (bad) {
-        if (tid == 0) { atomicAdd(B.status, 1); B.desc[tile] = make_int4(0, 0, 0, 0); }
-        for (int l = tid; l < LP; l += LT) {
-            B.r0[p0 + l] = 1.0; B.r1[p0 + l] = 1.0; B.gi[p0 + l] = 1.0; B.lid[p0 + l] = 0u; B.pos[p0 + l] = 0u;
-        }
-        return;
-    }
+            if (head[u]) B.tok[tile * LP + g] = (int32_t)sk[i];
+        }
+    }
+    if (tid == 0) s_ntok = ntok;
+    __syncthreads();
+    int s1[LI], p1[LI];
+#pragma unroll
+    for (int u = 0; u < LI; ++u) {
+        const int i = tid * LI + u;
+        s1[u] = (i < nh && (sv[i] >> 15)) ? 1 : 0;
+    }
+    Scan(tmp.scan).ExclusiveSum(s1, p1);
+#pragma unroll
+    for (int u = 0; u < LI; ++u) {
+        const int i = tid * LI + u;
+        if (i < nh) {
+            const uint32_t v = sv[i];
+            const int slot = v >> 15, l = v & 0x7fffu;
+            lidh[l][slot] = gid[i];
+            if (slot) { p1h[l] = (uint16_t)p1[u]; ftok[LP + p1[u]] = gid[i]; }
+            else ftok[l] = gid[i];
+        }
+    }
+    __syncthreads();
+    int hs[LI], rs[LI];
+#pragma unroll
+    for (int u = 0; u < LI; ++u) {
+        const int c = tid * LI + u;
+        hs[u] = (real(c) && (c == 0 || c == LP || ftok[c] != ftok[c - 1])) ? c : -1;
+    }
+    Scan(tmp.scan).InclusiveScan(hs, rs, MaxOp());
+#pragma unroll
+    for (int u = 0; u < LI; ++u) {
+        const int c = tid * LI + u;
+        if (real(c) && (c + 1 == LP || c + 1 == LH || !real(c + 1) || ftok[c + 1] != ftok[c])) rlen[rs[u]] = (uint16_t)(c - rs[u] + 1);
+    }
+    __syncthreads();
     const int cap = B.row_cap;
-    int nsub[2], rpre[2];
-#pragma unroll
-    for (int u = 0; u < 2; ++u) {
-        const int g = tid * 2 + u;
-        nsub[u] = g < ntok ? (gs[g + 1] - gs[g] + cap - 1) / cap : 0;
-    }
-    int nrow;
-    Scan(tmp.scan).ExclusiveSum(nsub, rpre, nrow);
-    __syncthreads();
-#pragma unroll
-    for (int u = 0; u < 2; ++u) {
-        const int g = tid * 2 + u;
-        if (g < ntok) {
-            rfirst[g] = rpre[u];
-            const int cnt = gs[g + 1] - gs[g];
-            for (int s = 0; s < nsub[u]; ++s) {
-                const int len = min(cap, cnt - cap * s);
-                rk[rpre[u] + s] = (uint32_t)(63 - len) << 16 | (uint32_t)(rpre[u] + s);
-            }
-        }
-    }
-    if (tid == 0) s_nrow = nrow;
-    __syncthreads();
     uint32_t rkey[LI], rdum[LI];
+    int nrow = 0;
+#pragma unroll
+    for (int u = 0; u < LI; ++u) {
+        const int c = tid * LI + u;
+        const int o = c - rs[u];
+        const bool rh = real(c) && o % cap == 0;
+        rkey[u] = rh ? (uint32_t)(63 - min(cap, (int)rlen[rs[u]] - o)) << 11 | (uint32_t)c : 0xffffffffu;
+        rdum[u] = 0u;
+        nrow += __syncthreads_count(rh);
+    }
+    if (nrow > LR) { inert_tile(B, tile); return; }
+    Sort(tmp.sort).Sort(rkey, rdum, 0, 17);
 #pragma unroll
     for (int u = 0; u < LI; ++u) {
         const int r = tid * LI + u;
-        rkey[u] = r < nrow ? rk[r] : 0xffffffffu;
-        rdum[u] = 0u;
-    }
-    __syncthreads();
-    Sort(tmp.sort).Sort(rkey, rdum, 0, 22);
-    int rlen[LI], spre[LI];
-#pragma unroll
-    for (int u = 0; u < LI; ++u) {
-        const int r = tid * LI + u;
-        rlen[u] = r < nrow ? 63 - (int)(rkey[u] >> 16) : 0;
-        if (r < nrow) rrank[rkey[u] & 0xffffu] = (uint16_t)r;
-    }
-    __syncthreads();
-    int total;
-    Scan(tmp.scan).ExclusiveSum(rlen, spre, total);
-#pragma unroll
-    for (int u = 0; u < LI; ++u) {
-        const int r = tid * LI + u;
-        if (r < nrow) { rstart[r] = spre[u]; rk[r] = (uint32_t)rlen[u]; }
-    }
-    __syncthreads();
-    for (int i = tid; i < nh; i += LT) {
-        const int g = gid[i], o = i - gs[g];
-        const int r = rrank[rfirst[g] + o / cap];
-        const int p = rstart[r] + o % cap;
-        const uint32_t v = sv[i];
-        const int slot = v >> 15, l = v & 0x7fffu;
-        lidh[l][slot] = (uint16_t)g;
-        posh[l][slot] = (uint16_t)p;
-        if (o % cap == 0) B.rows[tile * LR + r] = (uint32_t)rstart[r] | rk[r] << 16 | (uint32_t)g << 22;
-    }
-    __syncthreads();
+        if (r < nrow) {
+            const int c = (int)(rkey[u] & 0x7ffu);
+            B.rows[tile * LR + r] = (uint32_t)c | (uint32_t)(63 - (int)(rkey[u] >> 11)) << 16 | (uint32_t)ftok[c] << 22;
+        }
+    }
     for (int l = tid; l < LP; l += LT) {
         if (l < np) {
             const uint32_t pool = B.order[p0 + l];
-            B.lid[p0 + l] = (uint32_t)lidh[l][0] | (uint32_t)lidh[l][1] << 16;
-            B.pos[p0 + l] = (uint32_t)posh[l][0] | (uint32_t)posh[l][1] << 16;
+            B.pw[p0 + l] = (uint32_t)lidh[l][0] | (uint32_t)lidh[l][1] << 10 | (uint32_t)p1h[l] << 20;
             B.r0[p0 + l] = B.R[2 * (long long)pool]; B.r1[p0 + l] = B.R[2 * (long long)pool + 1];
             B.gi[p0 + l] = 1.0 / B.gamma[pool];
         } else {
-            const int pl = l - np;
-            B.lid[p0 + l] = 0u;
-            B.pos[p0 + l] = (uint32_t)(nh + 2 * pl) | (uint32_t)(nh + 2 * pl + 1) << 16;
+            B.pw[p0 + l] = (uint32_t)l << 20;
             B.r0[p0 + l] = 1.0; B.r1[p0 + l] = 1.0; B.gi[p0 + l] = 1.0;
         }
     }
-    if (tid == 0) { B.desc[tile] = make_int4(s_ntok, s_nrow, 0, 0); atomicAdd(B.status + 2, s_nrow); }
+    if (tid == 0) { B.desc[tile] = make_int4(s_ntok, nrow, 0, 0); atomicAdd(B.status + 2, nrow); }
 }
 
 inline size_t align_up(size_t x) { return (x + 255) & ~(size_t)255; }
@@ -224,7 +217,8 @@
     if (work_bytes < cfmm_blocked_build_work_bytes(n_pools)) return CFMM_E_SIZE;
     const long long T = (n_pools + LP - 1) / LP;
     if (out->pools_per_tile != LP || out->n_tiles != T || out->n_pools != n_pools) return CFMM_E_SIZE;
-    if (!out->r0 || !out->r1 || !out->gamma_inv || !out->lid || !out->pos || !out->rows || !out->tok || !out->desc) return CFMM_E_NULL;
+    if (!out->r0 || !out->r1 || !out->gamma_inv || !out->pw || !out->rows || !out->tok || !out->desc) return CFMM_E_NULL;
+    if (out->reserved_ptr) return CFMM_E_KIND;
     int row_cap = 32;
     cfmm_blocked_layout_info(nullptr, nullptr, nullptr, &row_cap);
     long long nb = (long long)llround(sqrt((double)n_pools / LP));
@@ -254,7 +248,7 @@
     B.m = n_pools; B.n_tokens = n_tokens; B.nb = (int)nb; B.row_cap = row_cap; B.key_bits = key_bits; B.tok_bits = 32;
     B.idx = idx; B.R = reserves; B.gamma = gamma; B.order = order;
     B.r0 = const_cast<double*>(out->r0); B.r1 = const_cast<double*>(out->r1); B.gi = const_cast<double*>(out->gamma_inv);
-    B.lid = const_cast<uint32_t*>(out->lid); B.pos = const_cast<uint32_t*>(out->pos);
+    B.pw = const_cast<uint32_t*>(out->pw);
     B.rows = const_cast<uint32_t*>(out->rows); B.tok = const_cast<int32_t*>(out->tok);
     B.desc = reinterpret_cast<int4*>(const_cast<int32_t*>(out->desc));
     B.status = status;
diff --git a/cfmm_routing_code_b200/pools.py b/cfmm_routing_code_b200/pools.py
--- a/cfmm_routing_code_b200/pools.py
+++ b/cfmm_routing_code_b200/pools.py
@@ -2,6 +2,7 @@
 
 import ctypes as C
 import dataclasses
+from collections.abc import Mapping
 from typing import Dict, List, Optional, Sequence
 
 import numpy as np
@@ -254,6 +255,73 @@
     return tuple(int(x.value) for x in v)
 
 
+def unpack_pool_words(pw: torch.Tensor, P: int):
+    w = pw.to(torch.int64) & 0xffffffff
+    l = torch.arange(w.numel(), device=w.device) % P
+    lid = (w & 0x3ff) | (((w >> 10) & 0x3ff) << 16)
+    pos = l | ((P + (w >> 20)) << 16)
+    return lid.to(torch.int32), pos.to(torch.int32)
+
+
+class BlockedTables(Mapping):
+    _DERIVED = ("lid", "pos")
+
+    def __init__(self, P: int, **tables):
+        self._P = P
+        self._t = tables
+
+    def __getitem__(self, k):
+        if k in self._DERIVED:
+            return unpack_pool_words(self._t["pw"], self._P)[self._DERIVED.index(k)]
+        return self._t[k]
+
+    def __iter__(self):
+        return iter(list(self._t) + list(self._DERIVED))
+
+    def __len__(self):
+        return len(self._t) + len(self._DERIVED)
+
+
+def _tile_layout(a: torch.Tensor, b: torch.Tensor, n_tokens: int, P: int, row_cap: int) -> dict:
+    dev = a.device
+    i64 = dict(dtype=torch.int64, device=dev)
+    mm = a.numel()
+    ntiles = -(-mm // P)
+    q = torch.arange(mm, **i64)
+    tile = q // P
+    ck, perm = torch.sort(torch.cat([tile, tile]) * n_tokens + torch.cat([a, b]), stable=True)
+    uniq, inv = torch.unique_consecutive(ck, return_inverse=True)
+    u_tile = uniq // n_tokens
+    ntok = torch.bincount(u_tile, minlength=ntiles)
+    ltok_u = torch.arange(uniq.numel(), **i64) - (torch.cumsum(ntok, 0) - ntok)[u_tile]
+    he_ltok = torch.empty(2 * mm, **i64)
+    he_ltok[perm] = ltok_u[inv]
+    lid0, lid1 = he_ltok[:mm], he_ltok[mm:]
+    s1 = torch.argsort(tile * n_tokens + b, stable=True)
+    p1 = torch.empty(mm, **i64)
+    p1[s1] = q - tile[s1] * P
+    F = torch.full((ntiles, 2 * P), -1, **i64)
+    F[tile, q - tile * P] = lid0
+    F[tile, P + p1] = lid1
+    F = F.view(-1)
+    c = torch.arange(F.numel(), **i64)
+    real = F >= 0
+    head = real & ((c % P == 0) | (F != torch.roll(F, 1)))
+    start = torch.cummax(torch.where(head, c, -1), 0).values
+    run = torch.cumsum(head.to(torch.int64), 0) - 1
+    run_len = torch.bincount(run[real])
+    o = c - start
+    rh = real & (o % row_cap == 0)
+    rc = c[rh]
+    row_len = torch.clamp(run_len[run[rh]] - o[rh], max=row_cap)
+    row_tile, row_start = rc // (2 * P), rc % (2 * P)
+    srt = torch.argsort((row_tile * 64 + (63 - row_len)) * (2 * P) + row_start)
+    row_tile, row_start, row_len, row_ltok = row_tile[srt], row_start[srt], row_len[srt], F[rc][srt]
+    nrow = torch.bincount(row_tile, minlength=ntiles)
+    return dict(ntiles=ntiles, ntok=ntok, nrow=nrow, uniq=uniq, u_tile=u_tile, ltok_u=ltok_u, lid0=lid0, lid1=lid1, p1=p1,
+                row_tile=row_tile, row_start=row_start, row_len=row_len, row_ltok=row_ltok)
+
+
 def build_blocked_pairs(idx: torch.Tensor, n_tokens: int, P: int, rows_stride: int, tok_stride: int, row_cap: int):
     dev = idx.device
     m = idx.shape[1]
@@ -267,71 +335,34 @@
         mm = order.numel()
         if mm == 0:
             break
-        pos = torch.arange(mm, **i64)
-        ntiles = -(-mm // P)
-        tile = pos // P
-        he_tok = torch.cat([a[order], b[order]])
-        he_tile = torch.cat([tile, tile])
-        ck, perm = torch.sort(he_tile * n_tokens + he_tok, stable=True)
-        uniq, inv, counts = torch.unique_consecutive(ck, return_inverse=True, return_counts=True)
-        u_tile = uniq // n_tokens
-        ntok = torch.bincount(u_tile, minlength=ntiles)
-        bad = ntok > tok_stride
+        L = _tile_layout(a[order], b[order], n_tokens, P, row_cap)
+        bad = (L["ntok"] > tok_stride) | (L["nrow"] > rows_stride)
         if not bool(bad.any()):
             break
         if _pass == 3:
             residual.append(order); order = order[:0]; mm = 0
             break
-        keep = ~bad[tile]
+        keep = ~bad[torch.arange(mm, **i64) // P]
         residual.append(order[~keep])
         order = order[keep]
     residual = torch.cat(residual) if residual else order[:0]
     if order.numel() == 0:
         return order, residual, None
-    U = uniq.numel()
-    tok_off = torch.cumsum(ntok, 0) - ntok
-    ltok_u = torch.arange(U, **i64) - tok_off[u_tile]
-    he_ltok = torch.empty(2 * mm, **i64)
-    he_ltok[perm] = ltok_u[inv]
+    ntiles, ntok, nrow = L["ntiles"], L["ntok"], L["nrow"]
     M = ntiles * P
-    lid = torch.zeros(M, dtype=torch.int32, device=dev)
-    lid[:mm] = (he_ltok[:mm] | (he_ltok[mm:] << 16)).to(torch.int32)
+    pw = (torch.arange(M, **i64) % P) << 20
+    pw[:mm] = L["lid0"] | (L["lid1"] << 10) | (L["p1"] << 20)
     tok = torch.zeros((ntiles, tok_stride), dtype=torch.int32, device=dev)
-    tok[u_tile, ltok_u] = (uniq - u_tile * n_tokens).to(torch.int32)
-    nsub = (counts + row_cap - 1) // row_cap
-    n_rows = int(nsub.sum())
-    first_row_u = torch.cumsum(nsub, 0) - nsub
-    row_u = torch.repeat_interleave(torch.arange(U, **i64), nsub)
-    sub = torch.arange(n_rows, **i64) - first_row_u[row_u]
-    g_start = torch.cumsum(counts, 0) - counts
-    row_tile0 = u_tile[row_u]
-    row_len0 = torch.clamp(counts[row_u] - row_cap * sub, max=row_cap)
-    srt = torch.argsort(row_tile0 * 64 + (63 - row_len0), stable=True)
-    rank = torch.empty_like(srt); rank[srt] = torch.arange(n_rows, **i64)
-    row_tile, row_len, row_ltok = row_tile0[srt], row_len0[srt], ltok_u[row_u][srt]
-    nrow = torch.bincount(row_tile, minlength=ntiles)
-    row_first = torch.cumsum(nrow, 0) - nrow
-    r_local = torch.arange(n_rows, **i64) - row_first[row_tile]
-    if int(nrow.max()) > rows_stride:
-        raise _lib.CfmmError("blocked layout: row table overflow (library/builder mismatch)")
-    cs = torch.cumsum(row_len, 0) - row_len
-    row_start = cs - cs[row_first][row_tile]
-    he_o = torch.arange(2 * mm, **i64) - g_start[inv]
-    he_row = rank[first_row_u[inv] + he_o // row_cap]
-    he_pos = torch.empty(2 * mm, **i64)
-    he_pos[perm] = row_start[he_row] + he_o % row_cap
-    pos = torch.zeros(M, dtype=torch.int32, device=dev)
-    pad_base = 2 * (mm - (ntiles - 1) * P)
-    if M > mm:
-        padl = torch.arange(M - mm, **i64)
-        pos[mm:] = ((pad_base + 2 * padl) | ((pad_base + 2 * padl + 1) << 16)).to(torch.int32)
-    pos[:mm] = (he_pos[:mm] | (he_pos[mm:] << 16)).to(torch.int32)
+    tok[L["u_tile"], L["ltok_u"]] = (L["uniq"] - L["u_tile"] * n_tokens).to(torch.int32)
+    row_tile = L["row_tile"]
+    n_rows = row_tile.numel()
+    r_local = torch.arange(n_rows, **i64) - (torch.cumsum(nrow, 0) - nrow)[row_tile]
     rows = torch.zeros((ntiles, rows_stride), dtype=torch.int32, device=dev)
-    word = row_start | (row_len << 16) | (row_ltok << 22)
+    word = L["row_start"] | (L["row_len"] << 16) | (L["row_ltok"] << 22)
     rows[row_tile, r_local] = torch.where(word >= 2 ** 31, word - 2 ** 32, word).to(torch.int32)
     desc = torch.stack([ntok, nrow, torch.zeros_like(ntok), torch.zeros_like(ntok)], 1).to(torch.int32).contiguous()
-    tables = dict(n_tiles=ntiles, M=M, lid=lid, tok=tok, pos=pos, rows=rows, desc=desc,
-                  rows_per_pool=n_rows / mm, tok_per_tile=float(ntok.double().mean()))
+    tables = BlockedTables(P, n_tiles=ntiles, M=M, pw=pw.to(torch.int32), tok=tok, rows=rows, desc=desc,
+                           rows_per_pool=n_rows / mm, tok_per_tile=float(ntok.double().mean()))
     return order, residual, tables
 
 
@@ -383,7 +414,7 @@
         self.r1 = slab(R[order, 1], 1.0)
         self.gamma_inv = slab(1.0 / gam[order], 1.0)
         self.c_blocked = _lib.BlockedPairs(self.m, t["n_tiles"], P, 0, self.r0.data_ptr(), self.r1.data_ptr(),
-                                           self.gamma_inv.data_ptr(), t["lid"].data_ptr(), t["pos"].data_ptr(),
+                                           self.gamma_inv.data_ptr(), t["pw"].data_ptr(), None,
                                            t["rows"].data_ptr(), t["tok"].data_ptr(), t["desc"].data_ptr())
 
     def _build_native(self, hp, spec, device, lib, P, rows_stride, tok_stride) -> bool:
@@ -402,7 +433,7 @@
         R = torch.from_numpy(hp.reserves[2 * lo:2 * hi]).to(device, non_blocking=True)
         gam = torch.from_numpy(hp.gamma[lo:hi]).to(device, non_blocking=True)
         slabs = torch.empty((3, M), **f64)
-        words = torch.empty((2, M), **i32)
+        pw = torch.empty(M, **i32)
         rows = torch.empty((T, rows_stride), **i32)
         tok = torch.empty((T, tok_stride), **i32)
         desc = torch.empty((T, 4), **i32)
@@ -412,8 +443,8 @@
         if nbytes <= 0:
             return False
         work = torch.empty(nbytes, dtype=torch.uint8, device=device)
-        cb = _lib.BlockedPairs(m, T, P, 0, slabs[0].data_ptr(), slabs[1].data_ptr(), slabs[2].data_ptr(), words[0].data_ptr(),
-                               words[1].data_ptr(), rows.data_ptr(), tok.data_ptr(), desc.data_ptr())
+        cb = _lib.BlockedPairs(m, T, P, 0, slabs[0].data_ptr(), slabs[1].data_ptr(), slabs[2].data_ptr(), pw.data_ptr(),
+                               None, rows.data_ptr(), tok.data_ptr(), desc.data_ptr())
         st = C.c_void_p(torch.cuda.current_stream(device).cuda_stream)
         rc = lib.cfmm_blocked_build(m, hp.n_tokens, idx.data_ptr(), R.data_ptr(), gam.data_ptr(), C.byref(cb), order.data_ptr(),
                                     status.data_ptr(), work.data_ptr(), nbytes, st)
@@ -431,8 +462,8 @@
         self.stride = M
         self.r0, self.r1, self.gamma_inv = slabs[0], slabs[1], slabs[2]
         self._keep = (idx, R, gam, work)
-        self.tables = dict(n_tiles=T, M=M, lid=words[0], pos=words[1], rows=rows, tok=tok, desc=desc,
-                           rows_per_pool=int(st_h[2]) / m, tok_per_tile=None)
+        self.tables = BlockedTables(P, n_tiles=T, M=M, pw=pw, tok=tok, rows=rows, desc=desc,
+                                    rows_per_pool=int(st_h[2]) / m, tok_per_tile=None)
         self.c_blocked = cb
         return True
 
@@ -451,7 +482,7 @@
     def bytes_resident(self) -> int:
         if self.tables is None:
             return 0
-        ts = [self.r0, self.r1, self.gamma_inv] + [self.tables[k] for k in ("lid", "tok", "pos", "rows", "desc")]
+        ts = [self.r0, self.r1, self.gamma_inv] + [self.tables[k] for k in ("pw", "tok", "rows", "desc")]
         return sum(x.numel() * x.element_size() for x in ts)
 
     def out_struct(self, trades: bool, hess: bool):
diff --git a/include/cfmm_b200.h b/include/cfmm_b200.h
--- a/include/cfmm_b200.h
+++ b/include/cfmm_b200.h
@@ -64,8 +64,8 @@
     const double* r0;
     const double* r1;
     const double* gamma_inv;
-    const uint32_t* lid;
-    const uint32_t* pos;
+    const uint32_t* pw;
+    const void* reserved_ptr;
     const uint32_t* rows;
     const int32_t* tok;
     const int32_t* desc;
```

New measurement: 58.77 billion (median of 6 runs). 5.4% higher.
